# dscripka/openWakeWord

Measured on NVIDIA H100. Metric: 80ms audio-frames/sec (concurrent streams), higher is better.
Workload: dtype f16 operands / f32 accumulate (mel, BN, LayerNorm, sigmoid in f32; heads' first layer as fp16 hi/lo split = f32-grade)

## Files before the change

openwakeword_b200/csrc/cnn_tc_inc.cu:

```cuda
#include "oww_internal.h"
#include "tc_common.cuh"
#include "mel_device.cuh"
#include <cmath>
#include <cstring>
#include <type_traits>

namespace {

constexpr int kIncEpiWarps = 16;
constexpr int kIncThreads = kIncEpiWarps * 32;
constexpr int kIncMaxG = 7;
constexpr int kMelNF = 2;

__device__ __forceinline__ __half2 u32_as_half2(uint32_t v) {
    return __halves2half2(__ushort_as_half((unsigned short)(v & 0xFFFFu)), __ushort_as_half((unsigned short)(v >> 16)));
}

struct IncArgs {
    IncPlan plan;
    const float* mel; const int* mel_count; int64_t mel_stride; int mel_mask; int back;
    const float* w0; const float* s0; const float* b0;
    const uint8_t* wblob;
    const uint4* tails_in; uint4* tails_out;
    float* emb;
    int B;
    const int* live_chunks; int live_min;
    long long* dbg_clock;
    int fused;
    const int16_t* pcm; int64_t pcm_stride;
    int16_t* tail; int* seen; float* mel_rw; int* mel_count_rw;
    const float* mel_window; const float2* mel_twiddle; const int* mel_start; const int* mel_len; const float* mel_w; int mel_kmax;
    float* feat_ring; int64_t feat_stride; int feat_mask; int* feat_count;
    const HeadDev* heads; int n_heads; int max_n_in;
    float* scores; int score_stride;
    int hring_off, hslot_bytes, hns;
    const Gate* gates; int n_gates;
    uint4* gx; LateLay gx_lay;
};

__device__ __forceinline__ int head_rows(int slot_bytes, int K, int D) {
    const int r = (slot_bytes / (D * 4)) & ~3;
    return r < K ? r : K;
}

template <int kNL>
__global__ void __launch_bounds__(kIncThreads, 1) tc_inc_kernel(const __grid_constant__ IncArgs a) {
    extern __shared__ __align__(128) uint8_t smem[];
    const IncPlan& P = a.plan;
    const int NL = kNL ? kNL : P.n_layers;
    const bool fused = kNL == OWW_N_CONV && a.fused;
    const int G = P.G;
    uint64_t* bars = reinterpret_cast<uint64_t*>(smem);
    float* s_l0 = reinterpret_cast<float*>(smem + 704);
    uint4* act0 = reinterpret_cast<uint4*>(smem + 2048);

    const int warp = __shfl_sync(0xffffffffu, (int)(threadIdx.x >> 5), 0);
    const int lane = threadIdx.x & 31;
    const uint32_t bar0 = smem_u32(bars);
    auto wfull = [&](int i) { return bar0 + 8u * i; };
    const uint32_t tails_bar = bar0 + 8u * 2;
    auto hfull = [&](int i) { return bar0 + 8u * (3 + i); };
    auto hempty = [&](int i) { return bar0 + 8u * (7 + i); };

    if (threadIdx.x == 0) {
        for (int i = 0; i < 2; ++i) mbar_init(wfull(i), 1);
        mbar_init(tails_bar, 1);
        for (int i = 0; i < 4; ++i) { mbar_init(hfull(i), 1); mbar_init(hempty(i), kIncEpiWarps); }
        asm volatile("fence.mbarrier_init.release.cluster;" ::: "memory");
    }
    for (int i = threadIdx.x; i < 9 * 24; i += kIncThreads) s_l0[i] = a.w0[i];
    if (threadIdx.x < 24) { s_l0[216 + threadIdx.x] = a.s0[threadIdx.x]; s_l0[240 + threadIdx.x] = a.b0[threadIdx.x]; }
    asm volatile("fence.proxy.async.shared::cta;" ::: "memory");
    __syncthreads();

    auto load_weights = [&](int l) {
        mbar_expect_tx(wfull(l & 1), (uint32_t)P.L[l].w_bytes);
        bulk_g2s(smem_u32(smem + P.L[l].w_smem), a.wblob + P.L[l].w_off, (uint32_t)P.L[l].w_bytes, wfull(l & 1));
    };
    if (threadIdx.x == 0 && (int)blockIdx.x < P.n_groups) { load_weights(1); load_weights(2); }
    pdl_wait();

    int hq_head = 0, hq_layer = 0, hq_row = 0, hchunk_p = 0;
    auto issue_head_chunk = [&]() -> bool {
        if (hq_head >= a.n_heads) return false;
        const HeadDev& H = a.heads[hq_head];
        const int slot = hchunk_p % a.hns;
        mbar_wait(hempty(slot), ((hchunk_p / a.hns) & 1) ^ 1);
        uint32_t bytes; const float* src;
        if (hq_layer == 0) {
            bytes = (uint32_t)(96 * H.dims[1]) * 4u;
            src = H.blob + H.w_off[0] + (int64_t)hq_row * 96 * H.dims[1];
            if (++hq_row == H.n_in) { hq_row = 0; hq_layer = 1; }
        } else {
            const int K = H.dims[hq_layer], D = H.dims[hq_layer + 1];
            const int rows = head_rows(a.hslot_bytes, K, D);
            bytes = ((uint32_t)(min(rows, K - hq_row) * D) * 4u + 15u) & ~15u;
            src = H.blob + H.w_off[hq_layer] + (int64_t)hq_row * D;
            if ((hq_row += rows) >= K) { hq_row = 0; ++hq_layer; }
        }
        if (hq_layer >= H.n_layers) { hq_layer = 0; ++hq_head; }
        mbar_expect_tx(hfull(slot), bytes);
        bulk_g2s(smem_u32(smem + a.hring_off + slot * a.hslot_bytes), src, bytes, hfull(slot));
        ++hchunk_p;
        return true;
    };

    const int et = threadIdx.x;
    uint32_t epar[2] = {0, 0};
    uint32_t epi_tails_par = 0, mma_tails_par = 0;
    uint32_t hf_par = 0; int hchunk_e = 0;
    for (int grp = blockIdx.x; grp < P.n_groups; grp += gridDim.x) {
        const uint4* tin = a.tails_in + (int64_t)grp * P.tail_units;
        uint4* tout = a.tails_out + (int64_t)grp * P.tail_units;
        int* s_cnt = reinterpret_cast<int*>(smem + 512);
        int* s_live = s_cnt + 16;
        float* s_mel = reinterpret_cast<float*>(smem + P.scratch_off + 6144);
        if (a.dbg_clock && blockIdx.x == 0 && grp == 0 && et == 0) a.dbg_clock[101] = clock64();
        named_bar_sync(2, kIncEpiWarps * 32);
        if (et < G) {
            const int b = grp * G + et;
            s_live[et] = b < a.B && (!a.live_chunks || a.live_chunks[b] >= a.live_min);
        }
        named_bar_sync(2, kIncEpiWarps * 32);
        if (fused) {
            uint8_t* sc = smem + P.scratch_off;
            float2* s_tw = reinterpret_cast<float2*>(sc);
            float* s_win = reinterpret_cast<float*>(sc + 4096);
            uint8_t* s_work = smem + 2048 + warp * (kMelNF * kMelFrameScratch);
            float* s_floor = s_mel + G * 256;
            int seen_v = 1;
            for (int i = et; i < 512; i += kIncEpiWarps * 32) { s_tw[i] = a.mel_twiddle[i]; s_win[i] = a.mel_window[i]; }
            if (et < G) {
                const int b = grp * G + et;
                s_cnt[et] = s_live[et] ? a.mel_count_rw[b] : 0;
                s_cnt[8 + et] = s_live[et] ? a.feat_count[b] : 0;
                seen_v = s_live[et] ? a.seen[b] : 1;
                s_live[8 + et] = s_live[et] && seen_v == 0;
            }
            named_bar_sync(2, kIncEpiWarps * 32);
            const int my_start = a.mel_start[lane], my_len = a.mel_len[lane];
            const float* my_w = a.mel_w + lane * OWW_MEL_MAXSUPPORT;
            for (int fi = warp * kMelNF; fi < G * 8; fi += kIncEpiWarps * kMelNF) {
                const int16_t* tl[kMelNF]; const int16_t* bd[kMelNF]; int fr[kMelNF]; float db[kMelNF];
#pragma unroll
                for (int i = 0; i < kMelNF; ++i) {
                    const int fj = fi + i < G * 8 ? fi + i : fi;
                    int b = grp * G + (fj >> 3);
                    if (b >= a.B) b = grp * G;
                    tl[i] = a.tail + (int64_t)b * OWW_TAIL; bd[i] = a.pcm + (int64_t)b * a.pcm_stride; fr[i] = fj & 7;
                }
                long long* st = (a.dbg_clock && blockIdx.x == 0 && grp == 0 && warp == 0 && fi == 0) ? a.dbg_clock + 92 : nullptr;
                mel_frames_db<kMelNF>(tl, OWW_TAIL, bd, fr, s_work, s_tw, s_win, a.mel_kmax, my_start, my_len, my_w, lane, db, st);
#pragma unroll
                for (int i = 0; i < kMelNF; ++i)
                    if (fi + i < G * 8) s_mel[(fi + i) * 32 + lane] = db[i];
            }
            named_bar_sync(2, kIncEpiWarps * 32);
            if (a.dbg_clock && blockIdx.x == 0 && grp == 0 && et == 0) a.dbg_clock[97] = clock64();
            constexpr int kTW = OWW_TAIL / 2;
            const bool al = ((size_t)a.pcm & 3) == 0 && (a.pcm_stride & 1) == 0;
            uint32_t tv[4]; int ti[4];
#pragma unroll
            for (int u = 0; u < 4; ++u) {
                const int i = et + u * kIncEpiWarps * 32;
                ti[u] = -1; tv[u] = 0;
                if (i < G * kTW) {
                    const int g = i / kTW, k = i - g * kTW, b = grp * G + g;
                    if (s_live[g]) {
                        const int16_t* src = a.pcm + (int64_t)b * a.pcm_stride + (OWW_SAMPLES_PER_CHUNK - OWW_TAIL) + 2 * k;
                        tv[u] = al ? __ldg(reinterpret_cast<const uint32_t*>(src))
                                   : ((uint32_t)(unsigned short)__ldg(src) | ((uint32_t)(unsigned short)__ldg(src + 1) << 16));
                        ti[u] = b * kTW + k;
                    }
                }
            }
            if (warp < G) {
                float m = -INFINITY;
                const int j0 = s_live[8 + warp] ? 3 : 0;
#pragma unroll
                for (int j = 0; j < 8; ++j) if (j >= j0) m = fmaxf(m, s_mel[warp * 256 + j * 32 + lane]);
#pragma unroll
                for (int o = 16; o > 0; o >>= 1) m = fmaxf(m, __shfl_xor_sync(0xffffffffu, m, o));
                if (lane == 0) s_floor[warp] = m - 80.0f;
            }
            named_bar_sync(2, kIncEpiWarps * 32);
            for (int i = et; i < G * 256; i += kIncEpiWarps * 32) {
                const int g = i >> 8, b = grp * G + g;
                float v = fmaxf(s_mel[i], s_floor[g]);
                v = v / 10.0f + 2.0f;
                const int fr = (i >> 5) & 7, skip = s_live[8 + g] ? 3 : 0;
                if (fr < skip) v = 1.0f;
                s_mel[i] = v;
                if (s_live[g] && fr >= skip)
                    a.mel_rw[(int64_t)b * a.mel_stride + (int64_t)((s_cnt[g] + fr - skip) & a.mel_mask) * 32 + (i & 31)] = v;
            }
#pragma unroll
            for (int u = 0; u < 4; ++u)
                if (ti[u] >= 0) reinterpret_cast<uint32_t*>(a.tail)[ti[u]] = tv[u];
            static_assert(kIncMaxG * (OWW_TAIL / 2) <= 4 * kIncEpiWarps * 32, "tail copy: four words per thread cover a group");
            if (grp + (int)gridDim.x < P.n_groups && et < G * 20) {
                const int g = et / 20, ln = et - g * 20, b = (grp + (int)gridDim.x) * G + g;
                if (b < a.B) asm volatile("prefetch.global.L2 [%0];" ::"l"(reinterpret_cast<const char*>(a.pcm + (int64_t)b * a.pcm_stride) + ln * 128));
            }
            if (et < G && s_live[et]) {
                const int b = grp * G + et;
                a.mel_count_rw[b] = oww_wrap_count(s_cnt[et] + (s_live[8 + et] ? 5 : 8));
                const int sn = seen_v + 1;
                a.seen[b] = sn > (1 << 30) ? (1 << 30) : sn;
            }
            named_bar_sync(2, kIncEpiWarps * 32);
        }
        for (int l = 0; l < NL; ++l) {
            const IncLayer& L = P.L[l];
            const bool to_global = kNL != OWW_N_CONV && l == NL - 1 && NL < OWW_N_CONV;
            if (a.dbg_clock && blockIdx.x == 0 && grp == 0 && et == 0) a.dbg_clock[l] = clock64();
            uint4* nx = act0 + L.nx_base;
            auto fill_tails_and_guards = [&]() {
                if (L.nx_tail_off >= 0 && et == 0) {
                    const uint32_t per_bytes = (uint32_t)(2 * G * L.nx_Wp) * 16u;
                    mbar_expect_tx(tails_bar, per_bytes * L.cg_out);
                    for (int pl = 0; pl < L.cg_out; ++pl)
                        bulk_g2s(smem_u32(nx + pl * L.nx_pitch + 1), tin + L.nx_tail_off + pl * (2 * G * L.nx_Wp), per_bytes, tails_bar);
                }
                if (!L.final && et < L.cg_out) nx[et * L.nx_pitch] = make_uint4(0, 0, 0, 0);
            };
            if (l > 0 && L.kh3) { mbar_wait(tails_bar, mma_tails_par); mma_tails_par ^= 1; }
            if (!L.pool_t) fill_tails_and_guards();
            else if (et < L.cg_out) (act0 + L.tmp_base)[et * L.tmp_pitch] = make_uint4(0, 0, 0, 0);

            if (l == 0) {
                const int Wp = 33, NP2 = 17;
                for (int q = et; q < 8 * G * NP2; q += kIncEpiWarps * 32) {
                    const int j = q % NP2, tg = q / NP2, g = tg % G, t = tg / G;
                    const int f0 = 2 * j;
                    const int b = grp * G + g;
                    uint4* o = nx + 1 + tg * Wp + f0;
                    const uint4 z = make_uint4(0, 0, 0, 0);
                    if (j == 16) { o[0] = z; o[L.nx_pitch] = z; o[2 * L.nx_pitch] = z; continue; }
                    if (!s_live[g]) {
                        o[0] = z; o[L.nx_pitch] = z; o[2 * L.nx_pitch] = z;
                        o[1] = z; o[L.nx_pitch + 1] = z; o[2 * L.nx_pitch + 1] = z;
                        continue;
                    }
                    const float* base = a.mel + (int64_t)b * a.mel_stride;
                    const int row0 = (fused ? s_cnt[g] - 2 : a.mel_count[b] - a.back - 10) + t;
                    float x[3][4];
#pragma unroll
                    for (int dt = 0; dt < 3; ++dt) {
                        const float* rp = (fused && t + dt >= 2) ? s_mel + (g * 8 + t + dt - 2) * 32
                                                                   : base + (int64_t)((row0 + dt) & a.mel_mask) * 32;
#pragma unroll
                        for (int i = 0; i < 4; ++i) {
                            const int ff = f0 + i - 1;
                            x[dt][i] = (ff >= 0 && ff < 32) ? rp[ff] : 0.f;
                        }
                    }
#pragma unroll
                    for (int pl = 0; pl < 3; ++pl) {
                        __half2 h0[4], h1[4];
#pragma unroll
                        for (int u = 0; u < 4; ++u) {
                            float v0[2], v1[2];
#pragma unroll
                            for (int e = 0; e < 2; ++e) {
                                const int c = pl * 8 + u * 2 + e;
                                float s0 = 0.f, s1 = 0.f;
#pragma unroll
                                for (int k = 0; k < 9; ++k) {
                                    const float w = s_l0[k * 24 + c];
                                    s0 = fmaf(x[k / 3][k % 3], w, s0);
                                    s1 = fmaf(x[k / 3][k % 3 + 1], w, s1);
                                }
                                const float sc = s_l0[216 + c], bi = s_l0[240 + c];
                                v0[e] = act(fmaf(fmaxf(s0, 0.f), sc, bi));
                                v1[e] = act(fmaf(fmaxf(s1, 0.f), sc, bi));
                            }
                            h0[u] = __floats2half2_rn(v0[0], v0[1]);
                            h1[u] = __floats2half2_rn(v1[0], v1[1]);
                        }
                        o[pl * L.nx_pitch] = *reinterpret_cast<uint4*>(h0);
                        o[pl * L.nx_pitch + 1] = *reinterpret_cast<uint4*>(h1);
                    }
                }
            } else {
                mbar_wait(wfull(l & 1), epar[l & 1]);
                epar[l & 1] ^= 1;
                const float* sb = reinterpret_cast<const float*>(smem + L.w_smem + 3 * L.cgp * L.np * 16);
                uint4* dst = L.pool_t ? (act0 + L.tmp_base) : nx;
                const int dpitch = L.pool_t ? L.tmp_pitch : L.nx_pitch;
                const int t_off_units = L.pool_t ? 0 : L.nx_t_off * G * L.Wp;
                const int n_t64 = (L.M + 63) / 64;
                const int tail_start = (L.T_out - 2) * G * L.Wp;
                const uint32_t wp_magic = 0xFFFFFFFFu / (uint32_t)L.Wp + 1u, g_magic = G > 1 ? 0xFFFFFFFFu / (uint32_t)G + 1u : 0u;
                const bool edbg = a.dbg_clock && blockIdx.x == 0 && grp == 0 && et == 0;
                long long e0 = 0;
                if (edbg) e0 = clock64();
                const int wg = warp >> 2, wq = warp & 3, q = lane & 3;
                const uint32_t w_addr = smem_u32(smem + L.w_smem);
                const uint32_t a_base = smem_u32(act0 + L.in_base);
                const int nq = L.cgp / 2;
                const uint32_t a_hi_pair = (uint32_t)make_desc(0, (uint32_t)L.in_pitch * 16u, 128u);
                const uint32_t a_hi_self = (uint32_t)make_desc(0, 0u, 128u);
                const uint64_t dhi = make_desc(0, 0u, 128u) & 0xFFFFFFFF00000000ull;
                const uint32_t b_lo0 = (uint32_t)make_desc(0, (uint32_t)L.np * 16u, 128u);
                const uint32_t a_unit0 = (a_base >> 4) + 1u;
                const uint32_t b_unit0 = w_addr >> 4;
                const uint32_t tap0 = (uint32_t)L.tap[0], tap1 = (uint32_t)L.tap[1], tap2 = (uint32_t)L.tap[2];
                const uint32_t pitch2 = 2u * (uint32_t)L.in_pitch, np2 = 2u * (uint32_t)L.np, tap_w = (uint32_t)(L.cgp * L.np);
                const int n_pair = L.cg_in / 2;
                const bool chained = (L.cg_in & 1) != 0;
                const int n_steps = chained ? 3 * n_pair + 2 : 3 * nq;
                const uint32_t a_cross = (uint32_t)make_desc(0, ((uint32_t)(L.cg_in - 1) * (uint32_t)L.in_pitch + tap0 - tap1) * 16u, 128u);
                const uint32_t last_plane = (uint32_t)(L.cg_in - 1) * (uint32_t)L.in_pitch;
                const int nc = L.np <= 48 ? L.np : L.np / 2;
                const int n_chunks = L.np / nc;
                const int n_items = n_t64 * n_chunks;
                const int lM = L.M, lWp = L.Wp, lW = L.W, lnp = L.np, lcg_out = L.cg_out, ltail = L.nx_tail_off;
                const bool lpool = L.pool_t != 0;
                const uint32_t lin_pitch = (uint32_t)L.in_pitch;
                const int tail_pitch = 2 * G * lWp;
                auto mma_item = [&](auto nc_const, auto ns_const, float* acc, int it) {
                    constexpr int NP = decltype(nc_const)::value;
                    constexpr int NS = decltype(ns_const)::value;
                    constexpr bool kChained = NS % 3 == 2;
                    constexpr int kPair = kChained ? (NS - 2) / 3 : NS / 3, kNq = NS / 3;
                    const int t64 = it / n_chunks, c0 = (it - t64 * n_chunks) * NP;
                    const uint32_t a_t0 = a_unit0 + (uint32_t)(t64 * 64);
                    const uint32_t b_unit = b_unit0 + (uint32_t)c0;
#pragma unroll
                    for (int s = 0; s < NS; ++s) {
                        uint32_t a_off, a_f, b_off;
                        if (kChained) {
                            const int k1 = s - kPair - 1, k2 = s - 2 * kPair - 1;
                            a_off = s < kPair ? tap0 + (uint32_t)s * pitch2
                                  : s == kPair ? tap1
                                  : k1 < kPair ? tap1 + lin_pitch + (uint32_t)k1 * pitch2
                                  : k2 < kPair ? tap2 + (uint32_t)k2 * pitch2
                                  : tap2 + last_plane;
                            a_f = s == kPair ? a_cross : (k2 >= kPair ? a_hi_self : a_hi_pair);
                            b_off = (uint32_t)s * np2;
                        } else {
                            const int j = s / kNq, qq = s - j * kNq;
                            a_off = (j == 0 ? tap0 : j == 1 ? tap1 : tap2) + (uint32_t)qq * pitch2;
                            a_f = a_hi_pair;
                            b_off = (uint32_t)j * tap_w + (uint32_t)qq * np2;
                        }
                        wg_mma<NP>(acc, dhi | a_f | ((a_t0 + a_off) & 0x3FFFu), dhi | b_lo0 | ((b_unit + b_off) & 0x3FFFu), s > 0);
                    }
                };
                auto epi_item = [&](auto nc_const, auto final_const, const float* acc, int it) {
                    constexpr int NP = decltype(nc_const)::value;
                    constexpr bool kFinal = decltype(final_const)::value;
                    const int t64 = it / n_chunks, c0 = (it - t64 * n_chunks) * NP;
#pragma unroll
                    for (int i = 0; i < 2; ++i) {
                        const int m = t64 * 64 + wq * 16 + (lane >> 2) + 8 * i;
                        if (m >= lM) continue;
                        const int tg = (int)__umulhi((uint32_t)m, wp_magic);
                        const int f = m - tg * lWp;
                        const int g = G > 1 ? tg - (int)__umulhi((uint32_t)tg, g_magic) * G : 0;
                        const bool live = s_live[g] != 0;
                        if constexpr (kFinal) {
                            if (f != 0 || !live) continue;
                            float* o = fused ? a.feat_ring + (int64_t)(grp * G + g) * a.feat_stride + (int64_t)(s_cnt[8 + g] & a.feat_mask) * 96
                                               : a.emb + (int64_t)(grp * G + g) * 96;
#pragma unroll
                            for (int j = 0; j < NP / 8; ++j) {
                                const int c = c0 + j * 8 + 2 * q;
                                float2 r;
                                r.x = fmaf(acc[4 * j + 2 * i], sb[c], sb[lnp + c]);
                                r.y = fmaf(acc[4 * j + 2 * i + 1], sb[c + 1], sb[lnp + c + 1]);
                                *reinterpret_cast<float2*>(o + c) = r;
                            }
                            continue;
                        }
                        const bool pad = f == lW;
                        uint4* d0 = dst + (1 + t_off_units + m);
                        const bool keep_tail = !lpool && ltail >= 0 && m >= tail_start && live;
                        uint4* t0 = tout + (ltail + (m - tail_start));
#pragma unroll
                        for (int j = 0; j < NP / 8; ++j) {
                            const int pl = c0 / 8 + j;
                            if (pl >= lcg_out) break;
                            const int c = pl * 8 + 2 * q;
                            const float y0 = act(fmaf(acc[4 * j + 2 * i], sb[c], sb[lnp + c]));
                            const float y1 = act(fmaf(acc[4 * j + 2 * i + 1], sb[c + 1], sb[lnp + c + 1]));
                            const __half2 h = __floats2half2_rn(y0, y1);
                            const uint32_t hw = pad ? 0u : *reinterpret_cast<const uint32_t*>(&h);
                            reinterpret_cast<uint32_t*>(d0 + pl * dpitch)[q] = hw;
                            if (keep_tail) reinterpret_cast<uint32_t*>(t0 + pl * tail_pitch)[q] = hw;
                            if (to_global) {
                                const __half2 lo = __floats2half2_rn(y0 - __low2float(h), y1 - __high2float(h));
                                reinterpret_cast<uint32_t*>(d0 + (lcg_out + pl) * dpitch)[q] = pad ? 0u : *reinterpret_cast<const uint32_t*>(&lo);
                            }
                        }
                    }
                };
                auto run_items = [&](auto nc_const, auto ns_const, auto final_const) {
                    constexpr int NP = decltype(nc_const)::value;
                    for (int it = wg; it < n_items; it += 4) {
                        float acc0[NP / 2];
                        wg_fence();
                        mma_item(nc_const, ns_const, acc0, it);
                        wg_commit();
                        wg_wait_all();
                        if (edbg && it == 0) a.dbg_clock[61 + l] = clock64() - e0;
                        epi_item(nc_const, final_const, acc0, it);
                    }
                };
                using std::integral_constant;
                const std::false_type planes;
                switch (n_steps * 256 + nc) {
                    case 5 * 256 + 32: run_items(integral_constant<int, 32>{}, integral_constant<int, 5>{}, planes); break;
                    case 5 * 256 + 48: run_items(integral_constant<int, 48>{}, integral_constant<int, 5>{}, planes); break;
                    case 9 * 256 + 48: run_items(integral_constant<int, 48>{}, integral_constant<int, 9>{}, planes); break;
                    case 9 * 256 + 40: run_items(integral_constant<int, 40>{}, integral_constant<int, 9>{}, planes); break;
                    case 14 * 256 + 40: run_items(integral_constant<int, 40>{}, integral_constant<int, 14>{}, planes); break;
                    case 14 * 256 + 48: run_items(integral_constant<int, 48>{}, integral_constant<int, 14>{}, planes); break;
                    case 18 * 256 + 48:
                        if (kNL == OWW_N_CONV && L.final) run_items(integral_constant<int, 48>{}, integral_constant<int, 18>{}, std::true_type{});
                        else run_items(integral_constant<int, 48>{}, integral_constant<int, 18>{}, planes);
                        break;
                    default: __trap();
                }
                if (edbg) a.dbg_clock[81 + l] = clock64() - e0;
                if (L.pool_t) {
                    named_bar_sync(2, kIncEpiWarps * 32);
                    if (!to_global) fill_tails_and_guards();
                    if (L.nx_tail_off >= 0 && L.nx_rows_new == 1) {
                        mbar_wait(tails_bar, epi_tails_par);
                        const int perrow = G * L.nx_Wp;
                        for (int i = et; i < L.cg_out * perrow; i += kIncEpiWarps * 32) {
                            const int pl = i / perrow, u = i - pl * perrow;
                            if (s_live[u / L.nx_Wp])
                                tout[L.nx_tail_off + pl * 2 * perrow + u] = nx[pl * L.nx_pitch + 1 + perrow + u];
                        }
                    }
                    const uint4* src = act0 + L.tmp_base;
                    const int T2 = L.T_out / L.pool_t;
                    const int per = T2 * G * L.nx_Wp;
                    const uint32_t per_magic = 0xFFFFFFFFu / (uint32_t)per + 1u, nwp_magic = 0xFFFFFFFFu / (uint32_t)L.nx_Wp + 1u;
                    const uint32_t gp_magic = G > 1 ? 0xFFFFFFFFu / (uint32_t)G + 1u : 0u;
                    for (int i = et; i < L.cg_out * per; i += kIncEpiWarps * 32) {
                        const int pl = per > 1 ? (int)__umulhi((uint32_t)i, per_magic) : i, p = i - pl * per;
                        const int tg = (int)__umulhi((uint32_t)p, nwp_magic), f = p - tg * L.nx_Wp;
                        const int t = G > 1 ? (int)__umulhi((uint32_t)tg, gp_magic) : tg, g = tg - t * G;
                        uint4 res = make_uint4(0, 0, 0, 0);
                        if (to_global) {
                            uint4 res_lo = make_uint4(0, 0, 0, 0);
                            if (f < L.nx_W) {
                                uint32_t bh[4] = {0, 0, 0, 0}, bl[4] = {0, 0, 0, 0};
                                bool first = true;
                                for (int da = 0; da < L.pool_t; ++da)
                                    for (int db = 0; db < L.pool_f; ++db) {
                                        const int at = 1 + ((t * L.pool_t + da) * G + g) * L.Wp + f * L.pool_f + db;
                                        const uint4 q = src[pl * L.tmp_pitch + at], ql = src[(L.cg_out + pl) * L.tmp_pitch + at];
                                        const uint32_t qh[4] = {q.x, q.y, q.z, q.w}, qq[4] = {ql.x, ql.y, ql.z, ql.w};
#pragma unroll
                                        for (int u = 0; u < 4; ++u) {
                                            const __half2 h2 = u32_as_half2(qh[u]), l2 = u32_as_half2(qq[u]);
                                            const __half2 b2 = u32_as_half2(bh[u]), c2 = u32_as_half2(bl[u]);
                                            const uint32_t m = first ? 0xFFFFFFFFu
                                                                     : (__hgt2_mask(h2, b2) | (__heq2_mask(h2, b2) & __hgt2_mask(l2, c2)));
                                            bh[u] = (qh[u] & m) | (bh[u] & ~m);
                                            bl[u] = (qq[u] & m) | (bl[u] & ~m);
                                        }
                                        first = false;
                                    }
                                res = make_uint4(bh[0], bh[1], bh[2], bh[3]);
                                res_lo = make_uint4(bl[0], bl[1], bl[2], bl[3]);
                            }
                            if (s_live[g]) {
                                const int64_t u = late_unit(a.gx_lay, pl, grp * G + g, t, f);
                                a.gx[u] = res;
                                a.gx[u + (int64_t)L.cg_out * a.gx_lay.units] = res_lo;
                            }
                            continue;
                        }
                        if (f < L.nx_W) {
                            __half2 mx[4];
                            bool first = true;
                            for (int da = 0; da < L.pool_t; ++da)
                                for (int db = 0; db < L.pool_f; ++db) {
                                    const uint4 q = src[pl * L.tmp_pitch + 1 + ((t * L.pool_t + da) * G + g) * L.Wp + f * L.pool_f + db];
                                    const __half2* hv = reinterpret_cast<const __half2*>(&q);
#pragma unroll
                                    for (int u = 0; u < 4; ++u) mx[u] = first ? hv[u] : __hmax2(mx[u], hv[u]);
                                    first = false;
                                }
                            res = *reinterpret_cast<uint4*>(mx);
                        }
                        nx[pl * L.nx_pitch + 1 + L.nx_t_off * G * L.nx_Wp + p] = res;
                        if (L.nx_tail_off >= 0 && s_live[g]) {
                            const int keep = T2 >= 2 ? 2 : 1;
                            if (t >= T2 - keep)
                                tout[L.nx_tail_off + pl * (2 * G * L.nx_Wp) + ((2 - keep + t - (T2 - keep)) * G + g) * L.nx_Wp + f] = res;
                        }
                    }
                }
            }
            if (L.nx_tail_off >= 0) epi_tails_par ^= 1;
            asm volatile("fence.proxy.async.shared::cta;" ::: "memory");
            named_bar_sync(1, kIncEpiWarps * 32);
            if (l > 0 && et == 0) {
                if (l + 2 < NL) load_weights(l + 2);
                else if (grp + (int)gridDim.x < P.n_groups) {
                    if (l == NL - 2 && (l & 1)) load_weights(1);
                    if (l == NL - 1) { if (l & 1) load_weights(1); load_weights(2); }
                }
            }
        }
        if (a.dbg_clock && blockIdx.x == 0 && grp == 0 && et == 0) a.dbg_clock[OWW_N_CONV] = clock64();
        if (fused) {
            named_bar_sync(2, kIncEpiWarps * 32);
            if (a.n_heads > 0) {
            if (et == 0) {
                hq_head = hq_layer = hq_row = 0;
                for (int i = 0; i < a.hns && issue_head_chunk(); ++i) {}
            }
            auto refill_head_ring = [&]() {
                while (hchunk_p < hchunk_e - 1 + max(a.hns, 2) && issue_head_chunk()) {}
            };
            const int NI = a.max_n_in;
            float* feats = reinterpret_cast<float*>(smem + 2048);
            float* red = feats + G * NI * 96;
            float* hA = red + 4 * G * 128;
            float* hB = hA + G * 256;
            for (int i0 = et; i0 < G * NI * 24; i0 += 4 * kIncEpiWarps * 32) {
                float4 v[4];
#pragma unroll
                for (int u = 0; u < 4; ++u) {
                    const int i = i0 + u * kIncEpiWarps * 32;
                    v[u] = make_float4(0.f, 0.f, 0.f, 0.f);
                    if (i < G * NI * 24) {
                        const int g = i / (NI * 24), r = (i / 24) % NI, c4 = (i % 24) * 4, b = grp * G + g;
                        if (s_live[g]) {
                            const int row = s_cnt[8 + g] + 1 - NI + r;
                            if (row >= 0) v[u] = __ldcg(reinterpret_cast<const float4*>(a.feat_ring + (int64_t)b * a.feat_stride + (int64_t)(row & a.feat_mask) * 96 + c4));
                        }
                    }
                }
#pragma unroll
                for (int u = 0; u < 4; ++u) {
                    const int i = i0 + u * kIncEpiWarps * 32;
                    if (i < G * NI * 24) *reinterpret_cast<float4*>(feats + i * 4) = v[u];
                }
            }
            named_bar_sync(2, kIncEpiWarps * 32);
            for (int hh = 0; hh < a.n_heads; ++hh) {
                const HeadDev& H = a.heads[hh];
                const int D1 = H.dims[1], off = NI - H.n_in;
                {
                    const int slice = et >> 7, d = et & 127;
                    float acc[kIncMaxG];
#pragma unroll
                    for (int g = 0; g < kIncMaxG; ++g) acc[g] = 0.f;
                    for (int c = 0; c < H.n_in; ++c) {
                        const int slot = hchunk_e % a.hns;
                        mbar_wait(hfull(slot), (hf_par >> slot) & 1u);
                        hf_par ^= 1u << slot;
                        ++hchunk_e;
                        if (d < D1) {
                            const float* wr = reinterpret_cast<const float*>(smem + a.hring_off + slot * a.hslot_bytes) + slice * 24 * D1 + d;
                            const float* xr = feats + (off + c) * 96 + slice * 24;
#pragma unroll 2
                            for (int k4 = 0; k4 < 24; k4 += 4) {
                                const float w0 = wr[(k4 + 0) * D1], w1 = wr[(k4 + 1) * D1];
                                const float w2 = wr[(k4 + 2) * D1], w3 = wr[(k4 + 3) * D1];
#pragma unroll
                                for (int g = 0; g < kIncMaxG; ++g)
                                    if (g < G) {
                                        const float4 x = *reinterpret_cast<const float4*>(xr + g * NI * 96 + k4);
                                        acc[g] = fmaf(x.x, w0, acc[g]);
                                        acc[g] = fmaf(x.y, w1, acc[g]);
                                        acc[g] = fmaf(x.z, w2, acc[g]);
                                        acc[g] = fmaf(x.w, w3, acc[g]);
                                    }
                            }
                        }
                        __syncwarp();
                        if (lane == 0) mbar_arrive(hempty(slot));
                        if (et == 0) refill_head_ring();
                    }
                    if (d < D1) {
#pragma unroll
                        for (int g = 0; g < kIncMaxG; ++g)
                            if (g < G) red[(slice * G + g) * 128 + d] = acc[g];
                    }
                }
                named_bar_sync(2, kIncEpiWarps * 32);
                for (int i = et; i < G * D1; i += kIncEpiWarps * 32) {
                    const int g = i / D1, d = i - g * D1;
                    float v = __ldg(H.blob + H.b_off[0] + d) + red[(0 * G + g) * 128 + d];
                    v += red[(1 * G + g) * 128 + d];
                    v += red[(2 * G + g) * 128 + d];
                    v += red[(3 * G + g) * 128 + d];
                    hA[g * 256 + d] = v;
                }
                named_bar_sync(2, kIncEpiWarps * 32);
                float* cur = hA; float* nxt = hB;
                for (int l = 0; l < H.n_layers; ++l) {
                    const int D = H.dims[l + 1], K = H.dims[l];
                    if (l > 0) {
                        const int rows = head_rows(a.hslot_bytes, K, D);
                        const int nown = min(4, max(0, (G * D - et + kIncEpiWarps * 32 - 1) / (kIncEpiWarps * 32)));
                        float accl[4]; int cxo[4], dd[4];
#pragma unroll
                        for (int j = 0; j < 4; ++j) {
                            const int i = j < nown ? et + j * kIncEpiWarps * 32 : 0;
                            const int g = i / D;
                            dd[j] = i - g * D; cxo[j] = g * 256; accl[j] = 0.f;
                        }
                        for (int k0 = 0; k0 < K; k0 += rows) {
                            const int r = min(rows, K - k0);
                            const int slot = hchunk_e % a.hns;
                            mbar_wait(hfull(slot), (hf_par >> slot) & 1u);
                            hf_par ^= 1u << slot;
                            ++hchunk_e;
                            const float* wr = reinterpret_cast<const float*>(smem + a.hring_off + slot * a.hslot_bytes);
#pragma unroll
                            for (int j = 0; j < 4; ++j) {
                                if (j >= nown) break;
                                const float* cx = cur + cxo[j] + k0;
                                const float* wc = wr + dd[j];
                                float sacc = accl[j];
#pragma unroll 8
                                for (int k = 0; k < r; ++k) sacc = fmaf(cx[k], wc[k * D], sacc);
                                accl[j] = sacc;
                            }
                            __syncwarp();
                            if (lane == 0) mbar_arrive(hempty(slot));
                            if (et == 0) refill_head_ring();
                        }
#pragma unroll
                        for (int j = 0; j < 4; ++j)
                            if (j < nown) nxt[cxo[j] + dd[j]] = accl[j] + __ldg(H.blob + H.b_off[l] + dd[j]);
                        named_bar_sync(2, kIncEpiWarps * 32);
                        float* t = cur; cur = nxt; nxt = t;
                    }
                    if (l < H.n_layers - 1) {
                        if (warp < G) {
                            float* row = cur + warp * 256;
                            if (H.layernorm) {
                                float sum = 0.f;
                                for (int d = lane; d < D; d += 32) sum += row[d];
#pragma unroll
                                for (int o = 16; o > 0; o >>= 1) sum += __shfl_xor_sync(0xffffffffu, sum, o);
                                const float mu = sum / (float)D;
                                float sq = 0.f;
                                for (int d = lane; d < D; d += 32) { const float c = row[d] - mu; sq = fmaf(c, c, sq); }
#pragma unroll
                                for (int o = 16; o > 0; o >>= 1) sq += __shfl_xor_sync(0xffffffffu, sq, o);
                                const float rstd = 1.0f / sqrtf(sq / (float)D + 1e-5f);
                                const float* gm = H.blob + H.g_off[l];
                                const float* hb = H.blob + H.h_off[l];
                                for (int d = lane; d < D; d += 32)
                                    row[d] = fmaxf((row[d] - mu) * rstd * __ldg(gm + d) + __ldg(hb + d), 0.f);
                            } else {
                                for (int d = lane; d < D; d += 32) row[d] = fmaxf(row[d], 0.f);
                            }
                        }
                        named_bar_sync(2, kIncEpiWarps * 32);
                    }
                }
                if (et < G && s_live[et]) {
                    const int n_out = H.dims[H.n_layers];
                    float* row = cur + et * 256;
                    if (H.final_act == 4) {
                        for (int d = 0; d < n_out; ++d) row[d] = fmaxf(row[d], 0.f);
                    } else if (H.final_act == 1) {
                        for (int d = 0; d < n_out; ++d) row[d] = 1.0f / (1.0f + expf(-row[d]));
                    } else if (H.final_act == 2 || H.final_act == 3) {
                        float m = -INFINITY;
                        for (int d = 0; d < n_out; ++d) {
                            if (H.final_act == 3) row[d] = fmaxf(row[d], 0.f);
                            m = fmaxf(m, row[d]);
                        }
                        float sum = 0.f;
                        for (int d = 0; d < n_out; ++d) { row[d] = expf(row[d] - m); sum += row[d]; }
                        for (int d = 0; d < n_out; ++d) row[d] = row[d] / sum;
                    }
                    float* o = a.scores + (int64_t)(grp * G + et) * a.score_stride + H.col0;
                    for (int d = 0; d < n_out; ++d) o[d] = row[d];
                }
                named_bar_sync(2, kIncEpiWarps * 32);
            }
            }
            if (et < G && s_live[et]) {
                if (a.n_heads > 0) {
                    float* o = a.scores + (int64_t)(grp * G + et) * a.score_stride;
                    for (int q = 0; q < a.n_gates; ++q)
                        if (o[a.gates[q].main_col] > a.gates[q].thr) o[a.gates[q].main_col] = o[a.gates[q].ver_col];
                }
                a.feat_count[grp * G + et] = oww_wrap_count(s_cnt[8 + et] + 1);
            }
            named_bar_sync(2, kIncEpiWarps * 32);
            if (a.dbg_clock && blockIdx.x == 0 && grp == 0 && et == 0) a.dbg_clock[102] = clock64();
        }
    }
}

__global__ void __launch_bounds__(256) tc_capture_kernel(const uint4* planes, int64_t plane_pitch, int T, int Wp, int cg,
                                                         int win0, int n_win, int stream0, const int* ids, int G, int tail_off,
                                                         int tail_units, uint4* tails) {
    const int per = 2 * Wp;
    const int64_t total = (int64_t)n_win * cg * per;
    for (int64_t i = (int64_t)blockIdx.x * 256 + threadIdx.x; i < total; i += (int64_t)gridDim.x * 256) {
        const int u = (int)(i % per);
        const int pl = (int)((i / per) % cg);
        const int w = (int)(i / ((int64_t)per * cg));
        const int r = u / Wp, f = u - r * Wp;
        const int b = ids ? ids[stream0 + w] : stream0 + w, grp = b / G, g = b - grp * G;
        const uint4 v = planes[(int64_t)pl * plane_pitch + kGuard + (int64_t)(win0 + w) * T * Wp + (int64_t)(T - 2 + r) * Wp + f];
        tails[(int64_t)grp * tail_units + tail_off + pl * (2 * G * Wp) + (r * G + g) * Wp + f] = v;
    }
}

}

int oww_inc_build_plan(oww_ctx* ctx, int G, int n_streams, int n_layers, IncPlan* out) {
    if (G < 1 || G > kIncMaxG) return oww_fail(ctx, OWW_EINVAL, "group size must be 1..%d", kIncMaxG);
    const int NL = n_layers;
    if (NL < 3 || NL > OWW_N_CONV || (NL < OWW_N_CONV && !ctx->conv[NL - 1].pool_t))
        return oww_fail(ctx, OWW_EINVAL, "fused-CNN plan: cannot cut after layer %d", NL - 1);
    constexpr int kTop = 227 * 1024;
    constexpr int kActBase = 2048;
    IncPlan P;
    std::memset(&P, 0, sizeof(P));
    P.G = G;
    P.n_groups = (n_streams + G - 1) / G;
    P.n_layers = NL;
    for (int l = 0; l < OWW_N_CONV; ++l) P.L[l].nx_tail_off = -1;
    int rows_new = 8, W = 32;
    int tail_units = 0;
    int x_units = 0, y_units = 0;
    size_t w_off = 0;
    auto pitch_of = [&](int rows, int wp) { return (1 + rows * G * wp + 7) & ~7; };
    auto need = [&](int buf, int units) { if (buf) { if (units > y_units) y_units = units; } else { if (units > x_units) x_units = units; } };
    int cur_buf = 0;
    int use_x[OWW_N_CONV] = {0}, use_y[OWW_N_CONV] = {0};
    for (int l = 0; l < NL; ++l) {
        const ConvLayer& C = ctx->conv[l];
        IncLayer& L = P.L[l];
        const bool cut = l == NL - 1 && NL < OWW_N_CONV;
        L.final = l == OWW_N_CONV - 1;
        L.kh3 = C.kh == 3 && l > 0;
        L.W = W; L.Wp = W + 1;
        L.cg_in = C.cin / 8; L.cgp = (L.cg_in + 1) & ~1; L.np = (C.cout + 15) & ~15; L.cg_out = C.cout / 8;
        L.pool_t = C.pool_t; L.pool_f = C.pool_f;
        auto use = [&](int buf, int units) { need(buf, units); int& u = buf ? use_y[l] : use_x[l]; if (units > u) u = units; };
        if (l == 0) {
            L.T_out = 8; L.M = 0;
        } else {
            L.in_buf = cur_buf;
            L.rows_in = rows_new + (L.kh3 ? 2 : 0);
            L.T_out = rows_new;
            L.M = L.T_out * G * L.Wp;
            L.in_pitch = P.L[l - 1].nx_pitch;
            use(L.in_buf, L.in_pitch * L.cg_in);
            if (L.kh3) { L.tap[0] = 0; L.tap[1] = G * L.Wp; L.tap[2] = 2 * G * L.Wp; }
            else { L.tap[0] = -1; L.tap[1] = 0; L.tap[2] = 1; }
            L.w_off = (int)w_off;
            L.w_bytes = 3 * L.cgp * L.np * 16 + 2 * L.np * 4;
            w_off += (size_t)((L.w_bytes + 127) & ~127);
        }
        const bool next_kh3 = !cut && l + 1 < OWW_N_CONV && ctx->conv[l + 1].kh == 3;
        int nrows = L.T_out, nW = W;
        if (L.pool_t) { nrows = L.T_out / L.pool_t; nW = W / L.pool_f; }
        L.nx_W = nW; L.nx_Wp = nW + 1; L.nx_rows_new = nrows;
        L.nx_t_off = (next_kh3 && !L.final) ? 2 : 0;
        L.out_buf = l == 0 ? 0 : (cur_buf ^ 1);
        L.nx_buf = (l == 0) ? 0 : (L.pool_t ? cur_buf : L.out_buf);
        L.nx_pitch = pitch_of(nrows + L.nx_t_off, L.nx_Wp);
        if (L.pool_t) { L.tmp_pitch = pitch_of(L.T_out, L.Wp); use(L.out_buf, L.tmp_pitch * L.cg_out * (cut ? 2 : 1)); }
        if (!L.final && !cut) use(L.nx_buf, L.nx_pitch * L.cg_out);
        L.nx_tail_off = -1;
        if (L.nx_t_off == 2) { L.nx_tail_off = tail_units; tail_units += L.cg_out * 2 * G * L.nx_Wp; }
        cur_buf = L.nx_buf;
        rows_new = nrows; W = nW;
    }
    P.tail_units = tail_units;
    P.x_units = (x_units + 7) & ~7; P.y_units = (y_units + 7) & ~7;
    int size_nx[OWW_N_CONV] = {0}, size_tmp[OWW_N_CONV] = {0}, xlive[OWW_N_CONV + 1];
    for (int l = 0; l < NL; ++l) {
        const IncLayer& L = P.L[l];
        const bool cut = l == NL - 1 && NL < OWW_N_CONV;
        size_nx[l] = (L.final || cut) ? 0 : L.nx_pitch * L.cg_out;
        size_tmp[l] = L.pool_t ? L.tmp_pitch * L.cg_out * (cut ? 2 : 1) : 0;
    }
    for (int l = 0; l <= OWW_N_CONV; ++l) xlive[l] = 0;
    for (int l = 0; l < NL; ++l) {
        const IncLayer& L = P.L[l];
        auto upd = [&](int cls, int sz) { if (cls == 0 && sz > xlive[l]) xlive[l] = sz; };
        if (l > 0) upd(L.in_buf, size_nx[l - 1]);
        if (L.pool_t) upd(L.out_buf, size_tmp[l]);
        upd(L.nx_buf, size_nx[l]);
    }
    auto r8 = [](int v) { return (v + 7) & ~7; };
    int act_high[OWW_N_CONV] = {0};
    for (int l = 0; l < NL; ++l) {
        IncLayer& L = P.L[l];
        L.in_base = l > 0 ? P.L[l - 1].nx_base : 0;
        L.tmp_base = (L.pool_t && L.out_buf == 1) ? r8(xlive[l]) : 0;
        L.nx_base = L.nx_buf == 1 ? r8(xlive[l] > xlive[l + 1] ? xlive[l] : xlive[l + 1]) : 0;
        int hi = 0;
        if (l > 0 && L.in_base + size_nx[l - 1] > hi) hi = L.in_base + size_nx[l - 1];
        if (L.pool_t && L.tmp_base + size_tmp[l] > hi) hi = L.tmp_base + size_tmp[l];
        if (L.nx_base + size_nx[l] > hi) hi = L.nx_base + size_nx[l];
        act_high[l] = kActBase + hi * 16;
    }
    auto wsz = [&](int l) { return l >= 1 && l < NL ? (P.L[l].w_bytes + 127) & ~127 : 0; };
    for (int l = 1; l < NL; ++l) {
        const int above = wsz(l + 1) > wsz(l - 1) ? wsz(l + 1) : wsz(l - 1);
        P.L[l].w_smem = (l & 1) ? kTop - wsz(l) : kTop - above - wsz(l);
    }
    for (int l = 1; l < NL; ++l) {
        int w_low = P.L[l].w_smem;
        if (l + 1 < NL && P.L[l + 1].w_smem < w_low) w_low = P.L[l + 1].w_smem;
        if (act_high[l] > w_low || act_high[l - 1] > P.L[l].w_smem)
            return oww_fail(ctx, OWW_EUNSUPPORTED, "fused-CNN smem plan does not fit at layer %d (G=%d)", l, G);
        if (l >= 2 && wsz(l) < wsz(l - 1)) return oww_fail(ctx, OWW_EUNSUPPORTED, "weight sizes must not shrink with depth");
    }
    if (NL == OWW_N_CONV) {
        int off = kActBase + r8(size_nx[0]) * 16;
        const int work_end = kActBase + kIncEpiWarps * kMelNF * kMelFrameScratch;
        if (work_end > off) off = (work_end + 127) & ~127;
        const int need_b = 6144 + G * 256 * 4 + 64;
        P.scratch_off = (off + need_b <= P.L[1].w_smem && off + need_b <= P.L[2].w_smem) ? off : 0;
    }
    P.w_total_bytes = (int)w_off;
    P.smem_bytes = kTop;
    *out = P;
    return OWW_OK;
}

int oww_inc_setup(oww_ctx* ctx, const float* h_blob) {
    IncPlan P;
    int rc = oww_inc_build_plan(ctx, 1, 1, OWW_N_CONV, &P);
    if (rc) return rc;
    std::vector<uint8_t> blob(P.w_total_bytes, 0);
    size_t off = 0;
    for (int li = 0; li < OWW_N_CONV; ++li) {
        const ConvLayer& C = ctx->conv[li];
        const size_t nw = (size_t)C.kh * C.kw * C.cin * C.cout;
        const float* w = h_blob + off; const float* sc = w + nw; const float* bi = sc + C.cout;
        off += nw + 2 * (size_t)C.cout;
        if (li == 0) continue;
        const IncLayer& L = P.L[li];
        const int sexp = oww_weight_scale_exponent(w, nw);
        const float up = std::ldexp(1.0f, sexp), down = std::ldexp(1.0f, -sexp);
        __half* hw = reinterpret_cast<__half*>(blob.data() + L.w_off);
        const int cg = L.cg_in;
        auto octet_at = [&](int j, int g) {
            if (!(cg & 1)) return j * L.cgp + g;
            if (j == 0) return g < cg - 1 ? g : cg;
            if (j == 1) return g == 0 ? cg - 1 : cg + g;
            return 2 * cg + g;
        };
        for (int j = 0; j < 3; ++j)
            for (int g = 0; g < cg; ++g)
                for (int n = 0; n < L.np; ++n)
                    for (int e = 0; e < 8; ++e) {
                        const int c = g * 8 + e;
                        const float v = (c < C.cin && n < C.cout) ? w[((size_t)j * C.cin + c) * C.cout + n] : 0.f;
                        hw[(((size_t)octet_at(j, g)) * L.np + n) * 8 + e] = __float2half_rn(v * up);
                    }
        float* sb = reinterpret_cast<float*>(blob.data() + L.w_off + (size_t)3 * L.cgp * L.np * 16);
        for (int n = 0; n < L.np; ++n) { sb[n] = n < C.cout ? sc[n] * down : 0.f; sb[L.np + n] = n < C.cout ? bi[n] : 0.f; }
    }
    if (!ctx->d_inc_w) OWW_CUDA(ctx, cudaMalloc(&ctx->d_inc_w, blob.size()));
    OWW_CUDA(ctx, cudaMemcpy(ctx->d_inc_w, blob.data(), blob.size(), cudaMemcpyHostToDevice));
    return OWW_OK;
}

int oww_inc_n_layers(const oww_ctx* ctx) {
    return (ctx->cfg.cnn_mode == OWW_CNN_TC_INCREMENTAL && ctx->split_from < OWW_N_CONV) ? ctx->split_from : OWW_N_CONV;
}

int oww_inc_alloc_streams(oww_ctx* ctx) {
    int best_g = 0; double best_cost = 0;
    for (int g = 1; g <= kIncMaxG; ++g) {
        IncPlan P;
        if (oww_inc_build_plan(ctx, g, ctx->n_streams, oww_inc_n_layers(ctx), &P) != OWW_OK) continue;
        const int rounds = (P.n_groups + ctx->sm_count - 1) / ctx->sm_count;
        const double cost = rounds * (50.0 + 6.5 * g);
        if (!best_g || cost < best_cost) { best_g = g; best_cost = cost; }
    }
    if (!best_g) return oww_fail(ctx, OWW_EUNSUPPORTED, "no feasible group size for the fused CNN kernel");
    ctx->err.clear();
    int rc = oww_inc_build_plan(ctx, best_g, ctx->n_streams, oww_inc_n_layers(ctx), &ctx->inc_plan);
    if (rc) return rc;
    const size_t bytes = (size_t)ctx->inc_plan.n_groups * ctx->inc_plan.tail_units * 16;
    for (int i = 0; i < 2; ++i) {
        cudaFree(ctx->d_inc_tails[i]); ctx->d_inc_tails[i] = nullptr;
        OWW_CUDA(ctx, cudaMalloc(&ctx->d_inc_tails[i], bytes));
        OWW_CUDA(ctx, cudaMemset(ctx->d_inc_tails[i], 0, bytes));
    }
    ctx->inc_cur = 0;
    ctx->tails_template_valid = false;
    OWW_CUDA(ctx, cudaFuncSetAttribute(tc_inc_kernel<OWW_N_CONV>, cudaFuncAttributeMaxDynamicSharedMemorySize, ctx->inc_plan.smem_bytes));
    OWW_CUDA(ctx, cudaFuncSetAttribute(tc_inc_kernel<11>, cudaFuncAttributeMaxDynamicSharedMemorySize, ctx->inc_plan.smem_bytes));
    OWW_CUDA(ctx, cudaFuncSetAttribute(tc_inc_kernel<15>, cudaFuncAttributeMaxDynamicSharedMemorySize, ctx->inc_plan.smem_bytes));
    OWW_CUDA(ctx, cudaFuncSetAttribute(tc_inc_kernel<0>, cudaFuncAttributeMaxDynamicSharedMemorySize, ctx->inc_plan.smem_bytes));
    return OWW_OK;
}

int oww_heads_sync_devs(oww_ctx* ctx) {
    std::vector<HeadDev> v(ctx->heads.size());
    for (size_t i = 0; i < ctx->heads.size(); ++i) {
        const Head& h = ctx->heads[i];
        HeadDev& d = v[i];
        std::memset(&d, 0, sizeof(d));
        d.blob = h.d_blob;
        d.n_in = h.desc.n_in; d.n_layers = h.desc.n_layers; d.layernorm = h.desc.layernorm; d.final_act = h.desc.final_act;
        for (int l = 0; l <= h.desc.n_layers; ++l) d.dims[l] = h.desc.dims[l];
        for (int l = 0; l < h.desc.n_layers; ++l) {
            d.w_off[l] = (int)h.w_off[l]; d.b_off[l] = (int)h.b_off[l];
            d.g_off[l] = (int)h.g_off[l]; d.h_off[l] = (int)h.h_off[l];
        }
        d.col0 = h.col0;
    }
    cudaFree(ctx->d_head_devs); ctx->d_head_devs = nullptr;
    if (v.empty()) return OWW_OK;
    OWW_CUDA(ctx, cudaMalloc(&ctx->d_head_devs, v.size() * sizeof(HeadDev)));
    OWW_CUDA(ctx, cudaMemcpy(ctx->d_head_devs, v.data(), v.size() * sizeof(HeadDev), cudaMemcpyHostToDevice));
    return OWW_OK;
}

bool oww_fused_frontend_supported(const oww_ctx* ctx) {
    return ctx->fuse_step && ctx->cfg.cnn_mode == OWW_CNN_TC_INCREMENTAL &&
           (ctx->inc_plan.n_layers < OWW_N_CONV || ctx->inc_plan.scratch_off != 0);
}

bool oww_fused_heads_supported(const oww_ctx* ctx) {
    if (!oww_fused_frontend_supported(ctx) || ctx->heads.empty() || ctx->heads.size() > 16) return false;
    if (ctx->inc_plan.n_layers < OWW_N_CONV) return false;
    {
        size_t w1 = 0;
        for (const Head& h : ctx->heads) w1 += (size_t)h.desc.dims[0] * h.desc.dims[1] * sizeof(float);
        if ((size_t)ctx->inc_plan.n_groups * w1 > ((size_t)256 << 20)) return false;
    }
    for (const Head& h : ctx->heads) {
        if (h.desc.dims[1] > 128) return false;
        for (int l = 1; l <= h.desc.n_layers; ++l) if (h.desc.dims[l] > 256) return false;
    }
    const size_t floats = (size_t)ctx->inc_plan.G * ((size_t)ctx->max_n_in * 96 + 4 * 128 + 2 * 256);
    int d1max = 32;
    for (const Head& h : ctx->heads) d1max = h.desc.dims[1] > d1max ? h.desc.dims[1] : d1max;
    return 2048 + floats * 4 + 128 + (size_t)96 * d1max * 4 <= (size_t)ctx->inc_plan.L[2].w_smem;
}

static cudaError_t launch_inc(const IncArgs& a, int grid, cudaStream_t s, bool pdl = false) {
    void (*k)(IncArgs) = a.plan.n_layers == OWW_N_CONV ? tc_inc_kernel<OWW_N_CONV>
                       : a.plan.n_layers == 11         ? tc_inc_kernel<11>
                       : a.plan.n_layers == 15         ? tc_inc_kernel<15>
                                                       : tc_inc_kernel<0>;
    return oww_launch_pdl(pdl, k, dim3(grid), dim3(kIncThreads), (size_t)a.plan.smem_bytes, s, a);
}

static void fill_inc_args(oww_ctx* ctx, IncArgs& a) {
    std::memset(&a, 0, sizeof(a));
    a.plan = ctx->inc_plan;
    a.mel = ctx->d_mel_ring; a.mel_count = ctx->d_mel_count; a.mel_stride = (int64_t)ctx->mel_rows * 32;
    a.mel_mask = ctx->mel_rows - 1;
    a.w0 = ctx->conv[0].d_w; a.s0 = ctx->conv[0].d_scale; a.b0 = ctx->conv[0].d_bias;
    a.wblob = reinterpret_cast<const uint8_t*>(ctx->d_inc_w);
    a.tails_in = reinterpret_cast<const uint4*>(ctx->d_inc_tails[ctx->inc_cur]);
    a.tails_out = reinterpret_cast<uint4*>(ctx->d_inc_tails[ctx->inc_cur ^ 1]);
    a.B = ctx->n_streams;
    a.dbg_clock = reinterpret_cast<long long*>(ctx->d_inc_dbg);
    if (ctx->late_active) {
        a.gx = reinterpret_cast<uint4*>(ctx->late_x[ctx->split_from].buf[0]);
        a.gx_lay = ctx->late_x[ctx->split_from].lay;
    }
}

int oww_fused_step(oww_ctx* ctx, const int16_t* d_pcm, int64_t pcm_stride, float* d_scores, int out_stride, bool with_heads,
                   cudaStream_t s, const int* d_chunks, int min_chunks) {
    IncArgs a;
    fill_inc_args(ctx, a);
    a.live_chunks = d_chunks; a.live_min = min_chunks;
    const int grid = a.plan.n_groups < ctx->sm_count ? a.plan.n_groups : ctx->sm_count;
    if (a.plan.n_layers < OWW_N_CONV) {
        MelLaunch m{d_pcm, pcm_stride, OWW_SAMPLES_PER_CHUNK, ctx->d_tail, ctx->d_seen, ctx->d_mel_ring,
                    (int64_t)ctx->mel_rows * 32, ctx->mel_rows - 1, ctx->d_mel_count, ctx->n_streams, 1, 1};
        m.live = d_chunks; m.live_min = min_chunks; m.pdl = ctx->late_pdl;
        int rc = oww_mel_launch(ctx, m, s);
        if (rc) return rc;
        OWW_CUDA(ctx, launch_inc(a, grid, s, ctx->late_pdl));
        OWW_LAUNCH_CHECK(ctx);
        ctx->inc_cur ^= 1;
        return OWW_OK;
    }
    a.fused = 1;
    a.pcm = d_pcm; a.pcm_stride = pcm_stride;
    a.tail = ctx->d_tail; a.seen = ctx->d_seen; a.mel_rw = ctx->d_mel_ring; a.mel_count_rw = ctx->d_mel_count;
    a.mel_window = ctx->d_window; a.mel_twiddle = ctx->d_twiddle; a.mel_start = ctx->d_mel_start; a.mel_len = ctx->d_mel_len;
    a.mel_w = ctx->d_mel_w; a.mel_kmax = ctx->mel_kmax;
    a.feat_ring = ctx->d_feat_ring; a.feat_stride = (int64_t)ctx->feat_rows * 96; a.feat_mask = ctx->feat_rows - 1;
    a.feat_count = ctx->d_feat_count;
    a.heads = ctx->d_head_devs; a.n_heads = with_heads ? (int)ctx->heads.size() : 0; a.max_n_in = ctx->max_n_in > 0 ? ctx->max_n_in : 1;
    a.scores = d_scores; a.score_stride = out_stride;
    a.gates = ctx->d_gates; a.n_gates = with_heads ? (int)ctx->gates.size() : 0;
    if (with_heads) {
        int d1max = 32;
        for (const Head& h : ctx->heads) d1max = h.desc.dims[1] > d1max ? h.desc.dims[1] : d1max;
        const int G = a.plan.G;
        const int used = 2048 + (G * (a.max_n_in * 96 + 4 * 128 + 2 * 256)) * 4;
        a.hring_off = (used + 127) & ~127;
        a.hslot_bytes = 96 * d1max * 4;
        const int avail = a.plan.L[2].w_smem - a.hring_off;
        a.hns = avail / a.hslot_bytes;
        if (a.hns > 4) a.hns = 4;
        if (a.hns < 1 && !ctx->heads.empty()) return oww_fail(ctx, OWW_EUNSUPPORTED, "no room for the fused heads weight ring");
    }
    OWW_CUDA(ctx, launch_inc(a, grid, s));
    OWW_LAUNCH_CHECK(ctx);
    ctx->inc_cur ^= 1;
    return OWW_OK;
}

int oww_cnn_inc_step(oww_ctx* ctx, int back, float* d_emb, cudaStream_t s, const int* d_chunks, int min_chunks) {
    IncArgs a;
    fill_inc_args(ctx, a);
    a.live_chunks = d_chunks; a.live_min = min_chunks;
    a.back = back;
    a.emb = d_emb;
    const int grid = a.plan.n_groups < ctx->sm_count ? a.plan.n_groups : ctx->sm_count;
    OWW_CUDA(ctx, launch_inc(a, grid, s));
    OWW_LAUNCH_CHECK(ctx);
    ctx->inc_cur ^= 1;
    if (ctx->late_active) return oww_late_chain(ctx, d_emb, s);
    return OWW_OK;
}

int oww_inc_capture(oww_ctx* ctx, int layer, const void* planes, int64_t plane_pitch, int T, int W, int win0, int n_win,
                    int stream0, const int* d_ids, cudaStream_t s) {
    const IncLayer& L = ctx->inc_plan.L[layer];
    if (layer >= ctx->inc_plan.n_layers - (ctx->inc_plan.n_layers < OWW_N_CONV ? 1 : 0) || L.nx_tail_off < 0) return OWW_OK;
    const int Wp = W + 1;
    const int64_t total = (int64_t)n_win * L.cg_out * 2 * Wp;
    unsigned grid = (unsigned)((total + 255) / 256);
    tc_capture_kernel<<<grid, 256, 0, s>>>(reinterpret_cast<const uint4*>(planes), plane_pitch, T, Wp, L.cg_out, win0, n_win,
                                          stream0, d_ids, ctx->inc_plan.G, L.nx_tail_off, ctx->inc_plan.tail_units,
                                          reinterpret_cast<uint4*>(ctx->d_inc_tails[ctx->inc_cur]));
    OWW_LAUNCH_CHECK(ctx);
    return OWW_OK;
}

namespace {
__global__ void fill_ones_kernel(float* p, int n) {
    const int i = blockIdx.x * blockDim.x + threadIdx.x;
    if (i < n) p[i] = 1.0f;
}
}

int oww_inc_build_template(oww_ctx* ctx) {
    if (!ctx->emb_loaded) return oww_fail(ctx, OWW_EINVAL, "embedding weights not loaded");
    if (!ctx->d_tc_act[0] || !ctx->d_inc_tails[0]) return oww_fail(ctx, OWW_EINVAL, "oww_set_streams has not been called");
    IncPlan P1;
    int rc = oww_inc_build_plan(ctx, 1, 1, ctx->inc_plan.n_layers, &P1);
    if (rc) return rc;
    ctx->n_tail_tab = 0;
    for (int l = 0; l < OWW_N_CONV; ++l)
        if (P1.L[l].nx_tail_off >= 0)
            ctx->tail_tab[ctx->n_tail_tab++] = make_int4(P1.L[l].nx_tail_off, ctx->inc_plan.L[l].nx_tail_off, P1.L[l].cg_out, P1.L[l].nx_Wp);
    cudaFree(ctx->d_tails_template); ctx->d_tails_template = nullptr;
    OWW_CUDA(ctx, cudaMalloc(&ctx->d_tails_template, (size_t)P1.tail_units * 16));
    OWW_CUDA(ctx, cudaMemset(ctx->d_tails_template, 0, (size_t)P1.tail_units * 16));
    float* d_ones = nullptr; float* d_emb = nullptr;
    OWW_CUDA(ctx, cudaMalloc(&d_ones, OWW_WINDOW_ROWS * 32 * sizeof(float)));
    OWW_CUDA(ctx, cudaMalloc(&d_emb, 96 * sizeof(float)));
    fill_ones_kernel<<<(OWW_WINDOW_ROWS * 32 + 255) / 256, 256>>>(d_ones, OWW_WINDOW_ROWS * 32);
    const IncPlan saved_plan = ctx->inc_plan;
    void* const saved_tails = ctx->d_inc_tails[ctx->inc_cur];
    ctx->inc_plan = P1;
    ctx->d_inc_tails[ctx->inc_cur] = ctx->d_tails_template;
    WindowSrc src{d_ones, (int64_t)OWW_WINDOW_ROWS * 32, nullptr, -1, 0, 0};
    TailCapture cap{0, 1, 0};
    cap.late = ctx->late_active;
    rc = oww_cnn_tc_pyramid_cap(ctx, src, 1, d_emb, &cap, nullptr);
    cudaError_t e = cudaDeviceSynchronize();
    ctx->inc_plan = saved_plan;
    ctx->d_inc_tails[ctx->inc_cur] = saved_tails;
    cudaFree(d_ones); cudaFree(d_emb);
    if (rc) return rc;
    if (e != cudaSuccess) return oww_fail(ctx, OWW_ECUDA, "tails template: %s", cudaGetErrorString(e));
    ctx->tails_template_valid = true;
    return OWW_OK;
}
```

openwakeword_b200/csrc/mel.cu:

```cuda
#include "oww_internal.h"
#include "tc_common.cuh"
#include "mel_device.cuh"
#include <climits>
#include <cmath>
#include <cstring>

namespace {

constexpr int kWarps = 8;
constexpr int kThreads = kWarps * 32;

struct MelDev {
    const float* window;
    const float2* twiddle;
    const int* mel_start;
    const int* mel_len;
    const float* mel_w;
    int kmax;
};

__global__ void __launch_bounds__(kThreads, 5) mel_kernel(MelLaunch p, MelDev c) {
    __shared__ __align__(16) uint8_t s_work[kWarps][kMelFrameScratch];
    __shared__ float2 s_tw[512];
    __shared__ float s_win[512];
    __shared__ float s_red[kWarps];

    pdl_trigger();
    const int clip = p.ids ? p.ids[blockIdx.x] : blockIdx.x;
    const int tid = threadIdx.x, lane = tid & 31, warp = tid >> 5;
    if (p.live && p.live[clip] < p.live_min) {
        pdl_wait();
        return;
    }

    for (int i = tid; i < 512; i += kThreads) { s_tw[i] = c.twiddle[i]; s_win[i] = c.window[i]; }

    const bool streaming = p.tail != nullptr;
    const int prefix = streaming ? OWW_TAIL : 0;
    const int seen0 = streaming ? p.seen[clip] : 0;
    const bool fresh = streaming && seen0 == 0;
    const int total = prefix + p.n_body;
    const int T = (total - OWW_FFT_N) / OWW_HOP + 1;
    const int f0 = fresh ? 3 : 0;
    const int nrows = T - f0;
    const bool one_pass = nrows <= kWarps;
    const int16_t* body = p.body + (int64_t)clip * p.body_stride;
    const int16_t* tail = streaming ? p.tail + (int64_t)clip * OWW_TAIL : nullptr;
    const int row0 = p.out_count ? p.out_count[clip] : 0;
    float* out = p.out + (int64_t)clip * p.out_stride;
    __syncthreads();

    const int my_start = c.mel_start[lane];
    const int my_len = c.mel_len[lane];
    const float* my_w = c.mel_w + lane * OWW_MEL_MAXSUPPORT;
    float vmax = -INFINITY, kept = 0.f;

    for (int f = f0 + warp; f < T; f += kWarps) {
        float db;
        mel_frames_db<1>(&tail, prefix, &body, &f, s_work[warp], s_tw, s_win, c.kmax, my_start, my_len, my_w, lane, &db);
        vmax = fmaxf(vmax, db);
        if (one_pass) { kept = db; continue; }
        pdl_wait();
        const int r = f - f0;
        const int slot = p.out_rows_mask >= 0 ? ((row0 + r) & p.out_rows_mask) : r;
        out[(int64_t)slot * OWW_MEL_BINS + lane] = db;
    }
#pragma unroll
    for (int o = 16; o > 0; o >>= 1) vmax = fmaxf(vmax, __shfl_xor_sync(0xffffffffu, vmax, o));
    if (lane == 0) s_red[warp] = vmax;
    __syncthreads();
    float m = s_red[0];
#pragma unroll
    for (int w = 1; w < kWarps; ++w) m = fmaxf(m, s_red[w]);
    const float floor_db = m - 80.0f;
    int16_t tv[(OWW_TAIL + kThreads - 1) / kThreads];
#pragma unroll
    for (int u = 0; u < (OWW_TAIL + kThreads - 1) / kThreads; ++u) {
        const int i = tid + u * kThreads;
        tv[u] = streaming && i < OWW_TAIL ? __ldg(body + (p.n_body - OWW_TAIL + i)) : (int16_t)0;
    }
    pdl_wait();
    if (one_pass) {
        if (warp < nrows) {
            float v = fmaxf(kept, floor_db);
            if (p.affine) v = v / 10.0f + 2.0f;
            const int slot = p.out_rows_mask >= 0 ? ((row0 + warp) & p.out_rows_mask) : warp;
            out[(int64_t)slot * OWW_MEL_BINS + lane] = v;
        }
    } else {
        for (int i = tid; i < nrows * OWW_MEL_BINS; i += kThreads) {
            const int r = i >> 5, col = i & 31;
            const int slot = p.out_rows_mask >= 0 ? ((row0 + r) & p.out_rows_mask) : r;
            float* q = out + (int64_t)slot * OWW_MEL_BINS + col;
            float v = fmaxf(__ldcg(q), floor_db);
            if (p.affine) v = v / 10.0f + 2.0f;
            *q = v;
        }
    }
    if (streaming) {
        int16_t* tw = p.tail + (int64_t)clip * OWW_TAIL;
#pragma unroll
        for (int u = 0; u < (OWW_TAIL + kThreads - 1) / kThreads; ++u)
            if (tid + u * kThreads < OWW_TAIL) tw[tid + u * kThreads] = tv[u];
        if (tid == 0) {
            p.out_count[clip] = oww_wrap_count(row0 + nrows);
            const int sn = seen0 + p.n_chunks;
            p.seen[clip] = sn > (1 << 30) ? (1 << 30) : sn;
        }
    }
}

__host__ __device__ __forceinline__ int clip_frame_step(int f) { return f < 5 ? 0 : (f - 5) / 8 + 1; }
__host__ __device__ __forceinline__ int clip_group(int f, int chunk) {
    return (int)oww_call_first_step(oww_call_of_step(clip_frame_step(f), chunk), chunk);
}
__host__ __device__ __forceinline__ int clip_first_group(int k0, int chunk) { return clip_group(8 * k0 > 71 ? 8 * k0 - 71 : 0, chunk); }

__global__ void __launch_bounds__(kThreads) mel_clip_kernel(const int16_t* pcm, const int64_t* clip_off, const int* clip_len, int pad,
                                                            int chunk, int k0, int k1, float* out, int64_t out_stride, MelDev c) {
    extern __shared__ __align__(16) uint8_t dyn[];
    float2 (*s_buf)[2][256] = reinterpret_cast<float2 (*)[2][256]>(dyn);
    float2* s_tw = reinterpret_cast<float2*>(dyn + kWarps * 2 * 256 * sizeof(float2));
    float* s_win = reinterpret_cast<float*>(s_tw + 512);
    float (*s_pow)[264] = reinterpret_cast<float (*)[264]>(s_win + 512);
    int16_t (*s_frame)[512] = reinterpret_cast<int16_t (*)[512]>(s_pow + kWarps);
    int* s_gmax = reinterpret_cast<int*>(s_frame + kWarps);
    const int clip = blockIdx.x;
    const int tid = threadIdx.x, lane = tid & 31, warp = tid >> 5;
    const int v0 = 8 * k0;
    const int g0 = clip_first_group(k0, chunk);
    const int f0 = g0 == 0 ? 0 : 8 * g0 - 3;
    const int n_frames = 8 * k1 - 3;
    for (int i = tid; i < 512; i += kThreads) { s_tw[i] = c.twiddle[i]; s_win[i] = c.window[i]; }
    for (int i = tid; i < k1 - g0; i += kThreads) s_gmax[i] = INT_MIN;
    const int16_t* body = pcm + clip_off[clip];
    const int n_samples = clip_len[clip];
    float* o = out + (int64_t)clip * out_stride;
    for (int i = tid; i < (71 - v0) * 32; i += kThreads) o[i] = 1.0f;
    __syncthreads();
    const int my_start = c.mel_start[lane];
    const int my_len = c.mel_len[lane];
    const float* my_w = c.mel_w + lane * OWW_MEL_MAXSUPPORT;
    auto enc = [](float v) { int i = __float_as_int(v); return i >= 0 ? i : i ^ 0x7FFFFFFF; };
    for (int f = f0 + warp; f < n_frames; f += kWarps) {
        for (int j = lane; j < 512; j += 32) {
            const int64_t p = (int64_t)f * OWW_HOP + j - pad;
            s_frame[warp][j] = (p >= 0 && p < n_samples) ? body[p] : (int16_t)0;
        }
        __syncwarp();
        const float db = mel_frame_db<false>(nullptr, 0, s_frame[warp], 0, s_buf[warp][0], s_buf[warp][1], s_pow[warp], s_tw, s_win, c.kmax,
                                      my_start, my_len, my_w, lane);
        if (71 + f >= v0) o[(int64_t)(71 + f - v0) * 32 + lane] = db;
        float m = db;
#pragma unroll
        for (int k = 16; k > 0; k >>= 1) m = fmaxf(m, __shfl_xor_sync(0xffffffffu, m, k));
        if (lane == 0) atomicMax(&s_gmax[clip_group(f, chunk) - g0], enc(m));
        __syncwarp();
    }
    __syncthreads();
    const int fw = max(f0, v0 - 71);
    for (int i = tid; i < (n_frames - fw) * 32; i += kThreads) {
        const int f = fw + (i >> 5);
        const int e = s_gmax[clip_group(f, chunk) - g0];
        const float gmax = __int_as_float(e >= 0 ? e : e ^ 0x7FFFFFFF);
        float* q = o + (int64_t)(71 + f - v0) * 32 + (i & 31);
        *q = fmaxf(*q, gmax - 80.0f) / 10.0f + 2.0f;
    }
}

double hz_to_mel(double f) {
    const double f_sp = 200.0 / 3.0, min_log_hz = 1000.0, min_log_mel = min_log_hz / f_sp;
    const double logstep = std::log(6.4) / 27.0;
    return f >= min_log_hz ? min_log_mel + std::log(f / min_log_hz) / logstep : f / f_sp;
}
double mel_to_hz(double m) {
    const double f_sp = 200.0 / 3.0, min_log_hz = 1000.0, min_log_mel = min_log_hz / f_sp;
    const double logstep = std::log(6.4) / 27.0;
    return m >= min_log_mel ? min_log_hz * std::exp(logstep * (m - min_log_mel)) : f_sp * m;
}

}

int oww_mel_launch(oww_ctx* ctx, const MelLaunch& p, cudaStream_t s) {
    if (!ctx->mel_loaded) return oww_fail(ctx, OWW_EINVAL, "mel constants not loaded");
    const int prefix = p.tail ? OWW_TAIL : 0;
    if (prefix + p.n_body < OWW_FFT_N) return oww_fail(ctx, OWW_EINVAL, "clip shorter than 512 samples");
    if (p.n_clips <= 0) return OWW_OK;
    MelDev c{ctx->d_window, ctx->d_twiddle, ctx->d_mel_start, ctx->d_mel_len, ctx->d_mel_w, ctx->mel_kmax};
    OWW_CUDA(ctx, oww_launch_pdl(p.pdl, mel_kernel, dim3(p.n_clips), dim3(kThreads), 0, s, p, c));
    OWW_LAUNCH_CHECK(ctx);
    return OWW_OK;
}

int oww_mel_clips_launch(oww_ctx* ctx, const int16_t* d_pcm, const int64_t* d_off, const int* d_len, int n_clips, int pad,
                         int chunk, int k0, int k1, float* d_out, int64_t out_stride, cudaStream_t s) {
    if (!ctx->mel_loaded) return oww_fail(ctx, OWW_EINVAL, "mel constants not loaded");
    if (n_clips <= 0 || k1 <= k0) return OWW_OK;
    if (k0 < 0 || k1 - k0 > 8192 || chunk < 1 || oww_call_first_step(oww_call_of_step(k1, chunk), chunk) != k1)
        return oww_fail(ctx, OWW_EINVAL, "step range [%d,%d) is not a bulk frontend segment", k0, k1);
    MelDev c{ctx->d_window, ctx->d_twiddle, ctx->d_mel_start, ctx->d_mel_len, ctx->d_mel_w, ctx->mel_kmax};
    const size_t smem = (size_t)kWarps * 2 * 256 * sizeof(float2) + 512 * sizeof(float2) + 512 * sizeof(float) +
                        (size_t)kWarps * 264 * sizeof(float) + (size_t)kWarps * 512 * sizeof(int16_t) +
                        (size_t)(k1 - clip_first_group(k0, chunk)) * sizeof(int);
    if (!ctx->mel_clip_attr_set) {
        OWW_CUDA(ctx, cudaFuncSetAttribute(mel_clip_kernel, cudaFuncAttributeMaxDynamicSharedMemorySize, 100 * 1024));
        ctx->mel_clip_attr_set = true;
    }
    mel_clip_kernel<<<n_clips, kThreads, smem, s>>>(d_pcm, d_off, d_len, pad, chunk, k0, k1, d_out, out_stride, c);
    OWW_LAUNCH_CHECK(ctx);
    return OWW_OK;
}

extern "C" int oww_load_mel(oww_ctx* ctx, const float* h_window512, const float* h_mel_fb) {
    if (!ctx) return OWW_EINVAL;
    OWW_CUDA(ctx, cudaSetDevice(ctx->device));
    const double kPi = 3.14159265358979323846;
    std::vector<float> win(512, 0.f);
    if (h_window512) {
        std::memcpy(win.data(), h_window512, 512 * sizeof(float));
    } else {
        for (int n = 0; n < 400; ++n) win[56 + n] = (float)(0.5 - 0.5 * std::cos(2.0 * kPi * n / 400.0));
    }
    std::vector<float2> tw(512);
    for (int k = 0; k < 512; ++k) {
        const double a = -2.0 * kPi * k / 512.0;
        tw[k] = make_float2((float)std::cos(a), (float)std::sin(a));
    }
    std::vector<float> fb(OWW_N_BINS * OWW_MEL_BINS);
    if (h_mel_fb) {
        std::memcpy(fb.data(), h_mel_fb, fb.size() * sizeof(float));
    } else {
        const int n_mels = OWW_MEL_BINS;
        std::vector<double> mel_f(n_mels + 2);
        const double m0 = hz_to_mel(60.0), m1 = hz_to_mel(3800.0);
        for (int i = 0; i < n_mels + 2; ++i) mel_f[i] = mel_to_hz(m0 + (m1 - m0) * i / (n_mels + 1));
        for (int k = 0; k < OWW_N_BINS; ++k) {
            const double ff = 8000.0 * k / 256.0;
            for (int i = 0; i < n_mels; ++i) {
                const double lower = (ff - mel_f[i]) / (mel_f[i + 1] - mel_f[i]);
                const double upper = (mel_f[i + 2] - ff) / (mel_f[i + 2] - mel_f[i + 1]);
                double w = lower < upper ? lower : upper;
                if (w < 0) w = 0;
                w *= 2.0 / (mel_f[i + 2] - mel_f[i]);
                fb[k * n_mels + i] = (float)w;
            }
        }
    }
    std::vector<int> st(OWW_MEL_BINS, 0), ln(OWW_MEL_BINS, 0);
    std::vector<float> mw(OWW_MEL_BINS * OWW_MEL_MAXSUPPORT, 0.f);
    int kmax = 0;
    for (int i = 0; i < OWW_MEL_BINS; ++i) {
        int lo = -1, hi = -1;
        for (int k = 0; k < OWW_N_BINS; ++k)
            if (fb[k * OWW_MEL_BINS + i] != 0.f) { if (lo < 0) lo = k; hi = k; }
        if (lo < 0) { st[i] = 0; ln[i] = 0; continue; }
        if (hi - lo + 1 > OWW_MEL_MAXSUPPORT)
            return oww_fail(ctx, OWW_EUNSUPPORTED, "mel filter %d spans %d FFT bins (max %d)", i, hi - lo + 1,
                            OWW_MEL_MAXSUPPORT);
        st[i] = lo; ln[i] = hi - lo + 1;
        for (int k = lo; k <= hi; ++k) mw[i * OWW_MEL_MAXSUPPORT + (k - lo)] = fb[k * OWW_MEL_BINS + i];
        if (hi + 1 > kmax) kmax = hi + 1;
    }
    ctx->mel_kmax = kmax;
    ctx->mel_key = oww_fnv1a(fb.data(), fb.size() * sizeof(float), oww_fnv1a(win.data(), win.size() * sizeof(float)));
    auto up = [&](void** d, const void* h, size_t bytes) -> cudaError_t {
        if (!*d) { cudaError_t e = cudaMalloc(d, bytes); if (e != cudaSuccess) return e; }
        return cudaMemcpy(*d, h, bytes, cudaMemcpyHostToDevice);
    };
    OWW_CUDA(ctx, up((void**)&ctx->d_window, win.data(), 512 * sizeof(float)));
    OWW_CUDA(ctx, up((void**)&ctx->d_twiddle, tw.data(), 512 * sizeof(float2)));
    OWW_CUDA(ctx, up((void**)&ctx->d_mel_start, st.data(), OWW_MEL_BINS * sizeof(int)));
    OWW_CUDA(ctx, up((void**)&ctx->d_mel_len, ln.data(), OWW_MEL_BINS * sizeof(int)));
    OWW_CUDA(ctx, up((void**)&ctx->d_mel_w, mw.data(), mw.size() * sizeof(float)));
    ctx->mel_loaded = true;
    return OWW_OK;
}
```

openwakeword_b200/csrc/mel_device.cuh:

```cuda
#pragma once
#include <cuda_runtime.h>
#include <cstdint>
#include "oww_internal.h"

namespace {

__device__ __forceinline__ float2 cmul(float2 a, float2 b) {
    return make_float2(__fmaf_rn(a.x, b.x, -__fmul_rn(a.y, b.y)), __fmaf_rn(a.x, b.y, __fmul_rn(a.y, b.x)));
}

template <bool kBodyGlobal = true>
__device__ __forceinline__ float mel_frame_db(const int16_t* tail, int prefix, const int16_t* body, int f, float2* a, float2* b,
                                              float* pw_buf, const float2* s_tw, const float* s_win, int kmax, int my_start,
                                              int my_len, const float* my_w, int lane) {
#pragma unroll
        for (int j = 0; j < 8; ++j) {
            const int n = lane + 32 * j;
            const int s0 = f * OWW_HOP + 2 * n;
            float x0, x1;
            if (s0 + 1 < prefix) { x0 = (float)tail[s0]; x1 = (float)tail[s0 + 1]; }
            else if (s0 >= prefix) {
                if (kBodyGlobal) { x0 = (float)__ldg(body + (s0 - prefix)); x1 = (float)__ldg(body + (s0 + 1 - prefix)); }
                else { x0 = (float)body[s0 - prefix]; x1 = (float)body[s0 + 1 - prefix]; }
            }
            else { x0 = (float)tail[s0]; x1 = kBodyGlobal ? (float)__ldg(body) : (float)body[0]; }
            a[n] = make_float2(__fmul_rn(x0, s_win[2 * n]), __fmul_rn(x1, s_win[2 * n + 1]));
        }
        __syncwarp();
#pragma unroll
        for (int Ns = 1; Ns < 256; Ns *= 4) {
            const int tstep = 128 / Ns;
#pragma unroll
            for (int jj = 0; jj < 2; ++jj) {
                const int j = lane + 32 * jj;
                const int k = j & (Ns - 1);
                float2 v0 = a[j];
                float2 v1 = cmul(a[j + 64], s_tw[k * tstep]);
                float2 v2 = cmul(a[j + 128], s_tw[2 * k * tstep]);
                float2 v3 = cmul(a[j + 192], s_tw[3 * k * tstep]);
                float2 a0 = make_float2(v0.x + v2.x, v0.y + v2.y);
                float2 a1 = make_float2(v0.x - v2.x, v0.y - v2.y);
                float2 a2 = make_float2(v1.x + v3.x, v1.y + v3.y);
                float2 d = make_float2(v1.x - v3.x, v1.y - v3.y);
                float2 a3 = make_float2(d.y, -d.x);
                const int dst = (j / Ns) * Ns * 4 + k;
                b[dst] = make_float2(a0.x + a2.x, a0.y + a2.y);
                b[dst + Ns] = make_float2(a1.x + a3.x, a1.y + a3.y);
                b[dst + 2 * Ns] = make_float2(a0.x - a2.x, a0.y - a2.y);
                b[dst + 3 * Ns] = make_float2(a1.x - a3.x, a1.y - a3.y);
            }
            __syncwarp();
            float2* t = a; a = b; b = t;
        }
        for (int k = lane; k < kmax; k += 32) {
            float pw;
            if (k == 256) {
                const float x = a[0].x - a[0].y;
                pw = __fmul_rn(x, x);
            } else {
                const float2 zk = a[k & 255];
                const float2 zc = a[(256 - k) & 255];
                const float2 xe = make_float2(0.5f * (zk.x + zc.x), 0.5f * (zk.y - zc.y));
                const float2 dd = make_float2(zk.x - zc.x, zk.y + zc.y);
                const float2 xo = make_float2(0.5f * dd.y, -0.5f * dd.x);
                const float2 t2 = cmul(s_tw[k], xo);
                const float re = __fadd_rn(xe.x, t2.x), im = __fadd_rn(xe.y, t2.y);
                pw = __fmaf_rn(re, re, __fmul_rn(im, im));
            }
            pw_buf[k] = pw;
        }
        __syncwarp();
        float acc = 0.f;
        for (int i = 0; i < my_len; ++i) acc = fmaf(pw_buf[my_start + i], my_w[i], acc);
        const float db = 10.0f * logf(fmaxf(acc, 1e-10f)) / logf(10.0f);
    return db;
}

#ifndef OWW_FFT_SWZ
#define OWW_FFT_SWZ 1
#endif
__device__ __forceinline__ int fswz(int e) {
#if OWW_FFT_SWZ
    return e ^ (((e >> 4) & 3) * 5);
#else
    return e;
#endif
}

constexpr int kMelFrameScratch = 2048 + 2048;
template <int NF>
__device__ __forceinline__ void mel_frames_db(const int16_t* const* tail, int prefix, const int16_t* const* body, const int* f,
                                              uint8_t* bufs, const float2* s_tw, const float* s_win, int kmax, int my_start,
                                              int my_len, const float* my_w, int lane, float* db, long long* stamps = nullptr) {
    float2* a[NF]; float2* b[NF]; float* pw[NF];
    if (stamps && lane == 0) stamps[0] = clock64();
#pragma unroll
    for (int i = 0; i < NF; ++i) {
        a[i] = reinterpret_cast<float2*>(bufs + i * kMelFrameScratch);
        b[i] = a[i] + 256;
        pw[i] = reinterpret_cast<float*>(b[i]);
    }
    bool al[NF];
#pragma unroll
    for (int i = 0; i < NF; ++i) al[i] = (((size_t)body[i] | (size_t)tail[i]) & 3) == 0 && (prefix & 1) == 0;
    uint32_t raw[8][NF];
#pragma unroll
    for (int j = 0; j < 8; ++j) {
        const int n = lane + 32 * j;
#pragma unroll
        for (int i = 0; i < NF; ++i) {
            const int s0 = f[i] * OWW_HOP + 2 * n;
            if (al[i]) {
                raw[j][i] = s0 + 1 < prefix ? *reinterpret_cast<const uint32_t*>(tail[i] + s0)
                                            : __ldg(reinterpret_cast<const uint32_t*>(body[i] + (s0 - prefix)));
            } else {
                unsigned short u0, u1;
                if (s0 + 1 < prefix) { u0 = (unsigned short)tail[i][s0]; u1 = (unsigned short)tail[i][s0 + 1]; }
                else if (s0 >= prefix) { u0 = (unsigned short)__ldg(body[i] + (s0 - prefix)); u1 = (unsigned short)__ldg(body[i] + (s0 + 1 - prefix)); }
                else { u0 = (unsigned short)tail[i][s0]; u1 = (unsigned short)__ldg(body[i]); }
                raw[j][i] = (uint32_t)u0 | ((uint32_t)u1 << 16);
            }
        }
    }
#pragma unroll
    for (int j = 0; j < 8; ++j) {
        const int n = lane + 32 * j;
        const float2 wn = *reinterpret_cast<const float2*>(s_win + 2 * n);
#pragma unroll
        for (int i = 0; i < NF; ++i) {
            const float x0 = (float)(short)(raw[j][i] & 0xFFFFu), x1 = (float)(short)(raw[j][i] >> 16);
            a[i][fswz(n)] = make_float2(__fmul_rn(x0, wn.x), __fmul_rn(x1, wn.y));
        }
    }
    __syncwarp();
    if (stamps && lane == 0) stamps[1] = clock64();
#pragma unroll
    for (int Ns = 1; Ns < 256; Ns *= 4) {
        const int tstep = 128 / Ns;
        float2 t1 = make_float2(1.f, 0.f), t2 = t1, t3 = t1;
        if (Ns > 1 && Ns <= 32) { const int k = lane & (Ns - 1); t1 = s_tw[k * tstep]; t2 = s_tw[2 * k * tstep]; t3 = s_tw[3 * k * tstep]; }
#pragma unroll
        for (int jj = 0; jj < 2; ++jj) {
            const int j = lane + 32 * jj;
            const int k = j & (Ns - 1);
            if (Ns > 32) { t1 = s_tw[k * tstep]; t2 = s_tw[2 * k * tstep]; t3 = s_tw[3 * k * tstep]; }
            const int dst = (j / Ns) * Ns * 4 + k;
            const int sj = fswz(j);
            const int d0 = fswz(dst), d1 = fswz(dst + Ns), d2 = fswz(dst + 2 * Ns), d3 = fswz(dst + 3 * Ns);
#pragma unroll
            for (int i = 0; i < NF; ++i) {
                const float2 v0 = a[i][sj];
                float2 v1 = a[i][sj + 64], v2 = a[i][sj + 128], v3 = a[i][sj + 192];
                if (Ns > 1) { v1 = cmul(v1, t1); v2 = cmul(v2, t2); v3 = cmul(v3, t3); }
                float2 a0 = make_float2(v0.x + v2.x, v0.y + v2.y);
                float2 a1 = make_float2(v0.x - v2.x, v0.y - v2.y);
                float2 a2 = make_float2(v1.x + v3.x, v1.y + v3.y);
                float2 d = make_float2(v1.x - v3.x, v1.y - v3.y);
                float2 a3 = make_float2(d.y, -d.x);
                b[i][d0] = make_float2(a0.x + a2.x, a0.y + a2.y);
                b[i][d1] = make_float2(a1.x + a3.x, a1.y + a3.y);
                b[i][d2] = make_float2(a0.x - a2.x, a0.y - a2.y);
                b[i][d3] = make_float2(a1.x - a3.x, a1.y - a3.y);
            }
        }
        __syncwarp();
#pragma unroll
        for (int i = 0; i < NF; ++i) { float2* t = a[i]; a[i] = b[i]; b[i] = t; }
    }
    if (stamps && lane == 0) stamps[2] = clock64();
    for (int k = lane; k < kmax; k += 32) {
#pragma unroll
        for (int i = 0; i < NF; ++i) {
            float p;
            if (k == 256) {
                const float x = a[i][fswz(0)].x - a[i][fswz(0)].y;
                p = __fmul_rn(x, x);
            } else {
                const float2 zk = a[i][fswz(k & 255)];
                const float2 zc = a[i][fswz((256 - k) & 255)];
                const float2 xe = make_float2(0.5f * (zk.x + zc.x), 0.5f * (zk.y - zc.y));
                const float2 dd = make_float2(zk.x - zc.x, zk.y + zc.y);
                const float2 xo = make_float2(0.5f * dd.y, -0.5f * dd.x);
                const float2 t2 = cmul(s_tw[k], xo);
                const float re = __fadd_rn(xe.x, t2.x), im = __fadd_rn(xe.y, t2.y);
                p = __fmaf_rn(re, re, __fmul_rn(im, im));
            }
            pw[i][k] = p;
        }
    }
    __syncwarp();
    if (stamps && lane == 0) stamps[3] = clock64();
    float acc[NF];
#pragma unroll
    for (int i = 0; i < NF; ++i) acc[i] = 0.f;
    for (int q = 0; q < my_len; q += 4) {
        const float4 w4 = __ldg(reinterpret_cast<const float4*>(my_w + q));
        const float w[4] = {w4.x, w4.y, w4.z, w4.w};
#pragma unroll
        for (int e = 0; e < 4; ++e)
            if (q + e < my_len) {
#pragma unroll
                for (int i = 0; i < NF; ++i) acc[i] = fmaf(pw[i][my_start + q + e], w[e], acc[i]);
            }
    }
#pragma unroll
    for (int i = 0; i < NF; ++i) db[i] = 10.0f * logf(fmaxf(acc[i], 1e-10f)) / logf(10.0f);
    __syncwarp();
    if (stamps && lane == 0) stamps[4] = clock64();
}

}
```

openwakeword_b200/csrc/oww_internal.h:

```cpp
#pragma once
#include <cuda_runtime.h>
#include <algorithm>
#include <cmath>
#include <cstdint>
#include <cstdio>
#include <string>
#include <utility>
#include <vector>
#include "owwb200.h"

__host__ __device__ inline int oww_scale_exponent_of_max(float amax, int lo = -8, int hi = 24) {
    if (!(amax > 0.f) || !(amax <= 3.402823466e38f)) return 0;
    int e;
    frexpf(amax, &e);
    e = 14 - e;
    return e < lo ? lo : (e > hi ? hi : e);
}
inline int oww_weight_scale_exponent(const float* w, size_t n) {
    float amax = 0.f;
    for (size_t i = 0; i < n; ++i) amax = std::fmax(amax, std::fabs(w[i]));
    return oww_scale_exponent_of_max(amax);
}

#define OWW_N_CONV 20
#define OWW_FFT_N 512
#define OWW_N_BINS 257
#define OWW_HOP 160
#define OWW_TAIL 480
#define OWW_MEL_MAXSUPPORT 32

struct ConvLayer {
    int kh, kw, cin, cout, pool_t, pool_f;
    int t_in, f_in;
    int t_out, f_out;
    float* d_w;
    float* d_scale;
    float* d_bias;
};

struct Head {
    oww_head_desc desc;
    int n_out;
    int col0;
    float* d_blob;
    std::vector<size_t> w_off, b_off, g_off, h_off;
    struct TcLayer { int K, D, Kp, NP; uint32_t w_off, w_bytes; float unscale; };
    bool tc_ok = false;
    void* d_w1_tc = nullptr;
    std::vector<TcLayer> tc_layers;
    std::vector<float> tc_w0_host;
};

struct LateLay {
    int S, T, Wq, kh3;
    int units;
    int64_t blk_stride;
};
#ifdef __CUDACC__
__host__ __device__ __forceinline__ int64_t late_unit(const LateLay& L, int plane, int stream, int row, int f) {
    const int blk = stream / L.S, sl = stream - blk * L.S;
    const int within = L.kh3 ? (row * L.S + sl) * L.Wq + f : 1 + (sl * L.T + row) * L.Wq + f;
    return (int64_t)blk * L.blk_stride + (int64_t)plane * L.units + within;
}
#endif

struct ResetLate {
    uint4* now;
    uint4* next;
    const uint4* tmpl;
    int Wp, n_planes;
    int off;
    LateLay lay;
};
struct ResetTails { uint4* tails; const uint4* tmpl; int G, tail_units, n_tab; int4 tab[OWW_N_CONV]; int n_late; ResetLate late[OWW_N_CONV]; };

struct Gate { int main_col, ver_col; float thr; };

struct VerifierBank {
    int head_id, col0, n_cols, n_in, capacity;
    int head_bank = -1;
    float thr;
    float* d_mean = nullptr;
    float* d_weight = nullptr;
    float* d_bias = nullptr;
    int* d_assign = nullptr;
    int clip_slot = -1;
};

struct HeadBank {
    Head shape;
    int capacity = 0;
    size_t w_bytes = 0;
    size_t p_floats = 0;
    std::vector<int> p_off;
    uint8_t* d_w = nullptr;
    float* d_p = nullptr;
    void* d_slots = nullptr;
    std::vector<uint8_t> h_slots;
    std::vector<uint8_t> loaded;
    int clip_slot = -1;
    std::vector<int> assign;
    int n_items = 0;
    int* d_table = nullptr;
    int* h_stage = nullptr;
    cudaEvent_t stage_ev = nullptr;
};

#define OWW_COUNT_WRAP (1 << 30)
#define OWW_COUNT_REBASE ((1 << 30) - (1 << 20))
#ifdef __CUDACC__
__device__ __forceinline__ int oww_wrap_count(int c) { return c >= OWW_COUNT_WRAP ? c - OWW_COUNT_REBASE : c; }
#endif

struct HeadDev {
    const float* blob;
    int n_in, n_layers, layernorm, final_act;
    int dims[OWW_MAX_HEAD_LAYERS + 1];
    int w_off[OWW_MAX_HEAD_LAYERS], b_off[OWW_MAX_HEAD_LAYERS], g_off[OWW_MAX_HEAD_LAYERS], h_off[OWW_MAX_HEAD_LAYERS];
    int col0;
};

struct IncLayer {
    int kh3, final;
    int W, Wp;
    int rows_in, T_out, M;
    int cg_in, cgp, np, cg_out;
    int in_buf, out_buf;
    int in_base, tmp_base, nx_base;
    int in_pitch;
    int tap[3];
    int pool_t, pool_f, tmp_pitch;
    int nx_buf, nx_pitch, nx_W, nx_Wp, nx_rows_new, nx_t_off, nx_tail_off;
    int w_off, w_bytes, w_smem;
};
struct IncPlan {
    int G, n_groups, tail_units, x_units, y_units, w_total_bytes, smem_bytes;
    int scratch_off;
    IncLayer L[OWW_N_CONV];
    int n_layers;
};

struct oww_ctx {
    oww_config cfg;
    int device = 0;
    int sm_count = 132;
    std::string err;
    uint64_t launches = 0;

    bool mel_loaded = false;
    float* d_window = nullptr;
    float2* d_twiddle = nullptr;
    int* d_mel_start = nullptr;
    int* d_mel_len = nullptr;
    float* d_mel_w = nullptr;
    int mel_kmax = 0;

    bool emb_loaded = false;
    ConvLayer conv[OWW_N_CONV];
    float* d_emb_blob = nullptr;

    std::vector<Head> heads;
    std::vector<HeadBank> head_banks;
    int n_out_total = 0;
    int max_n_in = 0;
    std::vector<Gate> gates;
    Gate* d_gates = nullptr;
    float* d_scores_tmp = nullptr;
    size_t scores_tmp_floats = 0;
    std::vector<VerifierBank> banks;
    int* d_assign_stage = nullptr;
    bool verifiers_on = true;
    cudaEvent_t ver_ev[2] = {nullptr, nullptr};
    double* d_fit_scratch = nullptr;
    size_t fit_scratch_doubles = 0;
    int64_t* d_fit_off = nullptr;
    size_t fit_off_cap = 0;
    int* d_load_slots = nullptr;
    size_t load_slots_cap = 0;
    bool fit_attr_set = false;

    int n_streams = 0;
    int mel_rows = 128;
    int feat_rows = 128;
    int16_t* d_tail = nullptr;
    int* d_seen = nullptr;
    int* d_mel_count = nullptr;
    int* d_feat_count = nullptr;
    float* d_mel_ring = nullptr;
    float* d_feat_ring = nullptr;

    int window_batch = 256;
    float* d_act[2] = {nullptr, nullptr};
    size_t act_floats = 0;
    float* d_emb_tmp = nullptr;
    size_t emb_tmp_floats = 0;

    void* d_tc_w = nullptr;
    float* d_tc_sb = nullptr;
    void* d_tc_w3 = nullptr;
    float* d_tc_sb3 = nullptr;
    int split_from = 11;
    size_t tc_w_off[OWW_N_CONV] = {0};
    size_t tc_sb_off[OWW_N_CONV] = {0};
    void* d_tc_act[2] = {nullptr, nullptr};
    size_t tc_act_units = 0;

    void* d_inc_w = nullptr;
    void* d_inc_tails[2] = {nullptr, nullptr};
    int inc_cur = 0;
    struct LateTensor { void* buf[3] = {nullptr, nullptr, nullptr}; int n_buf = 0, rows_new = 0, W = 0, cg = 0, tmpl_off = -1;
                        LateLay lay = {0, 0, 0, 0, 0, 0}; };
    LateTensor late_x[OWW_N_CONV];
    void* d_late_tmp = nullptr;
    void* d_late_template = nullptr;
    bool late_active = false;
    bool late_pdl = true;
    long late_step = 0;

    void* d_tails_template = nullptr;
    bool tails_template_valid = false;
    int4 tail_tab[OWW_N_CONV];
    int n_tail_tab = 0;
    int* d_reset_ids = nullptr;
    float* d_reset_init = nullptr;

    uint64_t mel_key = 0, emb_key = 0;
    int* d_state_ids = nullptr;
    int* d_state_rejected = nullptr;
    cudaEvent_t state_ev[2] = {nullptr, nullptr};
    IncPlan inc_plan;
    void* d_inc_dbg = nullptr;
    HeadDev* d_head_devs = nullptr;
    bool fuse_step = true;

    cudaStream_t own_stream = nullptr;
    cudaStream_t copy_stream = nullptr;
    struct HostSlot {
        int16_t* h_pcm = nullptr; int16_t* d_pcm = nullptr; size_t pcm_bytes = 0;
        float* h_scores = nullptr; float* d_scores = nullptr; size_t sc_bytes = 0;
        cudaEvent_t h2d_done = nullptr, done = nullptr;
        bool busy = false;
    } slot[2];
    int next_slot = 0;
    std::vector<int32_t> slot_chunks[2];

    static constexpr int kRagSlots = 4;
    int32_t* h_rag[kRagSlots] = {nullptr, nullptr, nullptr, nullptr};
    int32_t* d_rag[kRagSlots] = {nullptr, nullptr, nullptr, nullptr};
    cudaEvent_t rag_ev[kRagSlots] = {nullptr, nullptr, nullptr, nullptr};
    int rag_next = 0, rag_streams = 0;
    float* d_rag_scores = nullptr;
    size_t rag_scores_floats = 0;

    bool timing = false;
    std::vector<cudaEvent_t> ev;
    std::vector<uint8_t> ev_fused;
    int ev_slots = 0;
    long ev_steps = 0;

    bool heads_attr_set = false;
    bool heads_tc_attr_set = false;
    uint32_t tc_blk_attr_mask = 0;
    bool mel_clip_attr_set = false;
    uint32_t tc_attr_mask = 0;
    bool tc_heads = true;
    int* d_peer_err = nullptr;
    bool grp_heads = true;
    struct oww_heads_grp* heads_grp = nullptr;
    int tc_heads_terms = 3;
    struct oww_detector* det = nullptr;
    struct oww_audio* audio = nullptr;
    struct oww_ingest_state* ingest = nullptr;
    struct oww_clip_resampler* clip_rs = nullptr;
};

int oww_fail(oww_ctx* ctx, int code, const char* fmt, ...);
void oww_verifier_fit_free(oww_ctx* ctx);
inline uint64_t oww_fnv1a(const void* p, size_t bytes, uint64_t h = 14695981039346656037ull) {
    const unsigned char* c = static_cast<const unsigned char*>(p);
    for (size_t i = 0; i < bytes; ++i) h = (h ^ c[i]) * 1099511628211ull;
    return h;
}
#define OWW_CUDA(ctx, call)                                                                    \
    do {                                                                                       \
        cudaError_t e__ = (call);                                                              \
        if (e__ != cudaSuccess)                                                                \
            return oww_fail((ctx), OWW_ECUDA, "%s failed: %s (%s:%d)", #call,                  \
                            cudaGetErrorString(e__), __FILE__, __LINE__);                      \
    } while (0)
#ifdef __CUDACC__
template <typename... KArgs, typename... Args>
inline cudaError_t oww_launch_pdl(bool pdl, void (*kernel)(KArgs...), dim3 grid, dim3 block, size_t smem, cudaStream_t s, Args&&... args) {
    cudaLaunchConfig_t cfg = {};
    cfg.gridDim = grid; cfg.blockDim = block; cfg.dynamicSmemBytes = smem; cfg.stream = s;
    cudaLaunchAttribute at[1];
    at[0].id = cudaLaunchAttributeProgrammaticStreamSerialization;
    at[0].val.programmaticStreamSerializationAllowed = pdl ? 1 : 0;
    cfg.attrs = at; cfg.numAttrs = 1;
    return cudaLaunchKernelEx(&cfg, kernel, std::forward<Args>(args)...);
}
__device__ __forceinline__ void oww_pdl_sync() {
    asm volatile("griddepcontrol.launch_dependents;" ::: "memory");
    asm volatile("griddepcontrol.wait;" ::: "memory");
}
#endif

#define OWW_LAUNCH_CHECK(ctx)                                                                  \
    do {                                                                                       \
        (ctx)->launches++;                                                                     \
        cudaError_t e__ = cudaGetLastError();                                                  \
        if (e__ != cudaSuccess)                                                                \
            return oww_fail((ctx), OWW_ECUDA, "kernel launch failed: %s (%s:%d)",              \
                            cudaGetErrorString(e__), __FILE__, __LINE__);                      \
    } while (0)

#ifdef __CUDACC__
#define OWW_HD __host__ __device__ __forceinline__
#else
#define OWW_HD inline
#endif
OWW_HD int64_t oww_clip_calls(int64_t L, int c) { return L > c ? (L - 1) / c : 0; }
OWW_HD int64_t oww_call_first_step(int64_t j, int c) { return j * c / OWW_SAMPLES_PER_CHUNK; }
OWW_HD int64_t oww_call_of_step(int64_t s, int c) { return ((int64_t)OWW_SAMPLES_PER_CHUNK * (s + 1) + c - 1) / c - 1; }

struct MelLaunch {
    const int16_t* body; int64_t body_stride; int n_body;
    int16_t* tail;
    int* seen;
    float* out; int64_t out_stride; int out_rows_mask;
    int* out_count;
    int n_clips; int affine; int n_chunks;
    const int* ids = nullptr;
    const int* live = nullptr;
    int live_min = 0;
    bool pdl = false;
};
int oww_mel_launch(oww_ctx* ctx, const MelLaunch& p, cudaStream_t s);
int oww_mel_clips_launch(oww_ctx* ctx, const int16_t* d_pcm, const int64_t* d_off, const int* d_len, int n_clips, int pad,
                         int chunk, int k0, int k1, float* d_out, int64_t out_stride, cudaStream_t s);

struct WindowSrc {
    const float* base; int64_t stride;
    const int* count; int rows_mask;
    int n_streams; int n_chunks;
    const int* ids = nullptr;
};
int oww_feat_append(oww_ctx* ctx, const float* d_emb, int n_chunks, cudaStream_t s, const int* d_ids = nullptr, int n_ids = 0);
int oww_cnn_window(oww_ctx* ctx, const WindowSrc& src, int n_windows, float* d_emb, cudaStream_t s, bool capture_tails = false);
int oww_cnn_fp32_pyramid(oww_ctx* ctx, const WindowSrc& src, int n, int T0, float* d_emb, int out_rows, int stop_layer,
                         float* d_dbg, cudaStream_t s);

int oww_tc_pack_weights(oww_ctx* ctx, const float* h_blob);
size_t oww_tc_act_units(const oww_ctx* ctx, int n_windows);
size_t oww_tc_act_units_T(const oww_ctx* ctx, int n, int T0);
int oww_late_alloc(oww_ctx* ctx);
int oww_late_chain(oww_ctx* ctx, float* d_emb, cudaStream_t s);
int oww_late_capture(oww_ctx* ctx, int next_layer, const void* planes, int64_t plane_pitch, int T, int W, cudaStream_t s);
int oww_cnn_tc_pyramid(oww_ctx* ctx, const WindowSrc& src, int n, int T0, float* d_emb, int out_rows, int stop_layer,
                       float* d_dbg, cudaStream_t s);
struct TailCapture { int win0, n_win, stream0; const int* ids = nullptr; bool late = false; };
int oww_cnn_tc_pyramid_cap(oww_ctx* ctx, const WindowSrc& src, int n, float* d_emb, const TailCapture* cap, cudaStream_t s);

int oww_inc_build_plan(oww_ctx* ctx, int G, int n_streams, int n_layers, IncPlan* out);
int oww_inc_n_layers(const oww_ctx* ctx);
int oww_inc_setup(oww_ctx* ctx, const float* h_blob);
int oww_inc_alloc_streams(oww_ctx* ctx);
int oww_cnn_inc_step(oww_ctx* ctx, int back, float* d_emb, cudaStream_t s, const int* d_chunks = nullptr, int min_chunks = 0);
bool oww_fused_frontend_supported(const oww_ctx* ctx);
bool oww_fused_heads_supported(const oww_ctx* ctx);
int oww_fused_step(oww_ctx* ctx, const int16_t* d_pcm, int64_t pcm_stride, float* d_scores, int out_stride, bool with_heads,
                   cudaStream_t s, const int* d_chunks = nullptr, int min_chunks = 0);
int oww_heads_sync_devs(oww_ctx* ctx);
int oww_inc_capture(oww_ctx* ctx, int layer, const void* planes, int64_t plane_pitch, int T, int W, int win0, int n_win,
                    int stream0, const int* d_ids, cudaStream_t s);

struct FeatSrc {
    const float* base; int64_t stride;
    const int* count; int rows_mask;
    int back;
    int steps = 0, row0 = 0;
    const int* idx = nullptr;
};
#ifdef __CUDACC__
struct FeatRows { const float* base; int r0, mask; };
__device__ __forceinline__ FeatRows feat_rows(const FeatSrc& src, int n_in, int s) {
    if (src.count) return FeatRows{src.base + (int64_t)s * src.stride, src.count[s] - src.back - n_in, src.rows_mask};
    if (src.steps > 0) {
        const int q = src.idx ? src.idx[s] : s;
        const int clip = q / src.steps, st = q - clip * src.steps;
        return FeatRows{src.base + (int64_t)clip * src.stride, src.row0 + st + 1 - n_in, -1};
    }
    return FeatRows{src.base + (int64_t)s * src.stride, 0, -1};
}
__device__ __forceinline__ const float* feat_row(const FeatRows& w, int c) {
    const int r = w.r0 + c;
    return r < 0 ? nullptr : w.base + (int64_t)(w.mask >= 0 ? (r & w.mask) : r) * 96;
}
#endif
int oww_heads_launch(oww_ctx* ctx, int head_id, const FeatSrc& src, int n, float* d_out, int out_stride,
                     int out_col0, int combine_max, cudaStream_t s, uint32_t head_mask = 0xFFFFFFFFu);

int oww_check_head_desc(oww_ctx* ctx, const oww_head_desc* desc);
int oww_stage_head(oww_ctx* ctx, const oww_head_desc* desc, const float* h_blob, size_t n_floats, Head& h,
                   std::vector<float>& staged);

int oww_heads_tc_pack(oww_ctx* ctx, Head& h, const float* w1);
struct BankRows { const int4* items; const int* perm; int n_items; };
int oww_head_banks_launch(oww_ctx* ctx, const FeatSrc& src, int n, float* d_out, int out_stride, int combine_max,
                          cudaStream_t s, const int* d_step = nullptr, const BankRows* rows = nullptr);
const int* oww_head_bank_stream_slots(const oww_ctx* ctx, int bank);
int oww_head_banks_alloc_streams(oww_ctx* ctx);
void oww_head_banks_free(oww_ctx* ctx);
bool oww_heads_tc_supported(const oww_ctx* ctx, int head_id);
int oww_heads_tc_launch(oww_ctx* ctx, int head_id, const FeatSrc& src, int n, float* d_out, int out_stride,
                        int out_col0, int combine_max, cudaStream_t s, uint32_t head_mask = 0xFFFFFFFFu);
void oww_heads_grp_free(oww_ctx* ctx);
void oww_heads_grp_drop_mirror(oww_ctx* ctx);
void oww_feat16_invalidate(oww_ctx* ctx);
int oww_feat16_advance(oww_ctx* ctx, int n_chunks, cudaStream_t s);
int oww_feat16_resync(oww_ctx* ctx, const int* d_ids, int n, cudaStream_t s);
uint32_t oww_heads_grp_covered(oww_ctx* ctx);
uint32_t oww_heads_grp_bulk(oww_ctx* ctx, const FeatSrc& src, int n, float* d_out, int out_stride, cudaStream_t s, int* rc_out);
int oww_heads_grp_launch(oww_ctx* ctx, int back, int n, float* d_out, int out_stride, int combine_max, cudaStream_t s);
int oww_heads_all(oww_ctx* ctx, const FeatSrc& src, int n, float* d_out, int out_stride, int combine_max, cudaStream_t s,
                  const BankRows* bank_rows = nullptr);

void oww_detect_free(oww_ctx* ctx);
void oww_detect_free_streams(oww_ctx* ctx);
int oww_detect_alloc_streams(oww_ctx* ctx);
int oww_detect_reset(oww_ctx* ctx, const int* d_ids, int n, cudaStream_t s);

void oww_audio_free(oww_ctx* ctx);
void oww_audio_free_streams(oww_ctx* ctx);
int oww_audio_alloc_streams(oww_ctx* ctx);
int oww_audio_reset(oww_ctx* ctx, const int* d_ids, int n, cudaStream_t s);
int oww_audio_append(oww_ctx* ctx, const int16_t* d_pcm, int64_t pcm_stride, int n_chunks, const int* d_counts,
                     cudaStream_t s);

void oww_ingest_free(oww_ctx* ctx);
void oww_ingest_free_streams(oww_ctx* ctx);
int oww_ingest_alloc_streams(oww_ctx* ctx);
void oww_ingest_reset(oww_ctx* ctx, const int32_t* h_ids, int n);

int oww_verifiers_apply(oww_ctx* ctx, const FeatSrc& src, int n, float* d_scores, int out_stride, bool clips,
                        cudaStream_t s, const int* d_chunks = nullptr, const int* d_clip_streams = nullptr);
int oww_verifiers_alloc_streams(oww_ctx* ctx);
bool oww_verifiers_clip_active(const oww_ctx* ctx, bool clip_streams = false);
void oww_verifiers_free_streams(oww_ctx* ctx);
```

Measured before the change: 6.238 million.

## Replace shared-memory mel FFT with register/shuffle FFT and pack clips per CTA

The 512-point real FFT used for mel frames now runs in registers with warp shuffles (radix-8 in-thread, then xor-shuffle stages) instead of radix-4 passes through shared memory. Per-lane window and twiddle values are preloaded and mel weights are transposed for coalesced loads. The standalone mel kernel is restructured into a persistent grid that packs several clips per CTA, with an occupancy-derived split of frames across warps. This targets shared-memory traffic, syncwarps and launch/occupancy overhead in the mel frontend, at the cost of more registers per thread and a changed weight and twiddle layout.

```diff
diff --git a/openwakeword_b200/csrc/cnn_tc_inc.cu b/openwakeword_b200/csrc/cnn_tc_inc.cu
--- a/openwakeword_b200/csrc/cnn_tc_inc.cu
+++ b/openwakeword_b200/csrc/cnn_tc_inc.cu
@@ -10,7 +10,6 @@
 constexpr int kIncEpiWarps = 16;
 constexpr int kIncThreads = kIncEpiWarps * 32;
 constexpr int kIncMaxG = 7;
-constexpr int kMelNF = 2;
 
 __device__ __forceinline__ __half2 u32_as_half2(uint32_t v) {
     return __halves2half2(__ushort_as_half((unsigned short)(v & 0xFFFFu)), __ushort_as_half((unsigned short)(v >> 16)));
@@ -114,7 +113,7 @@
         uint4* tout = a.tails_out + (int64_t)grp * P.tail_units;
         int* s_cnt = reinterpret_cast<int*>(smem + 512);
         int* s_live = s_cnt + 16;
-        float* s_mel = reinterpret_cast<float*>(smem + P.scratch_off + 6144);
+        float* s_mel = reinterpret_cast<float*>(smem + P.scratch_off);
         if (a.dbg_clock && blockIdx.x == 0 && grp == 0 && et == 0) a.dbg_clock[101] = clock64();
         named_bar_sync(2, kIncEpiWarps * 32);
         if (et < G) {
@@ -123,13 +122,9 @@
         }
         named_bar_sync(2, kIncEpiWarps * 32);
         if (fused) {
-            uint8_t* sc = smem + P.scratch_off;
-            float2* s_tw = reinterpret_cast<float2*>(sc);
-            float* s_win = reinterpret_cast<float*>(sc + 4096);
-            uint8_t* s_work = smem + 2048 + warp * (kMelNF * kMelFrameScratch);
+            float* s_pw = reinterpret_cast<float*>(smem + 2048 + warp * kMelPwBytes);
             float* s_floor = s_mel + G * 256;
             int seen_v = 1;
-            for (int i = et; i < 512; i += kIncEpiWarps * 32) { s_tw[i] = a.mel_twiddle[i]; s_win[i] = a.mel_window[i]; }
             if (et < G) {
                 const int b = grp * G + et;
                 s_cnt[et] = s_live[et] ? a.mel_count_rw[b] : 0;
@@ -139,21 +134,15 @@
             }
             named_bar_sync(2, kIncEpiWarps * 32);
             const int my_start = a.mel_start[lane], my_len = a.mel_len[lane];
-            const float* my_w = a.mel_w + lane * OWW_MEL_MAXSUPPORT;
-            for (int fi = warp * kMelNF; fi < G * 8; fi += kIncEpiWarps * kMelNF) {
-                const int16_t* tl[kMelNF]; const int16_t* bd[kMelNF]; int fr[kMelNF]; float db[kMelNF];
-#pragma unroll
-                for (int i = 0; i < kMelNF; ++i) {
-                    const int fj = fi + i < G * 8 ? fi + i : fi;
-                    int b = grp * G + (fj >> 3);
-                    if (b >= a.B) b = grp * G;
-                    tl[i] = a.tail + (int64_t)b * OWW_TAIL; bd[i] = a.pcm + (int64_t)b * a.pcm_stride; fr[i] = fj & 7;
-                }
+            const float* my_w = a.mel_w + lane;
+            const MelLane L = mel_lane_load(a.mel_window, a.mel_twiddle, lane);
+#pragma unroll 1
+            for (int fi = warp; fi < G * 8; fi += kIncEpiWarps) {
+                int b = grp * G + (fi >> 3);
+                if (b >= a.B) b = grp * G;
                 long long* st = (a.dbg_clock && blockIdx.x == 0 && grp == 0 && warp == 0 && fi == 0) ? a.dbg_clock + 92 : nullptr;
-                mel_frames_db<kMelNF>(tl, OWW_TAIL, bd, fr, s_work, s_tw, s_win, a.mel_kmax, my_start, my_len, my_w, lane, db, st);
-#pragma unroll
-                for (int i = 0; i < kMelNF; ++i)
-                    if (fi + i < G * 8) s_mel[(fi + i) * 32 + lane] = db[i];
+                s_mel[fi * 32 + lane] = mel_frame(L, a.tail + (int64_t)b * OWW_TAIL, OWW_TAIL, a.pcm + (int64_t)b * a.pcm_stride,
+                                                  fi & 7, s_pw, a.mel_kmax, my_start, my_len, my_w, lane, st);
             }
             named_bar_sync(2, kIncEpiWarps * 32);
             if (a.dbg_clock && blockIdx.x == 0 && grp == 0 && et == 0) a.dbg_clock[97] = clock64();
@@ -823,9 +812,9 @@
     }
     if (NL == OWW_N_CONV) {
         int off = kActBase + r8(size_nx[0]) * 16;
-        const int work_end = kActBase + kIncEpiWarps * kMelNF * kMelFrameScratch;
+        const int work_end = kActBase + kIncEpiWarps * kMelPwBytes;
         if (work_end > off) off = (work_end + 127) & ~127;
-        const int need_b = 6144 + G * 256 * 4 + 64;
+        const int need_b = G * 256 * 4 + 64;
         P.scratch_off = (off + need_b <= P.L[1].w_smem && off + need_b <= P.L[2].w_smem) ? off : 0;
     }
     P.w_total_bytes = (int)w_off;
diff --git a/openwakeword_b200/csrc/mel.cu b/openwakeword_b200/csrc/mel.cu
--- a/openwakeword_b200/csrc/mel.cu
+++ b/openwakeword_b200/csrc/mel.cu
@@ -9,6 +9,7 @@
 
 constexpr int kWarps = 8;
 constexpr int kThreads = kWarps * 32;
+constexpr int kKeep = 8;
 
 struct MelDev {
     const float* window;
@@ -19,93 +20,89 @@
     int kmax;
 };
 
-__global__ void __launch_bounds__(kThreads, 5) mel_kernel(MelLaunch p, MelDev c) {
-    __shared__ __align__(16) uint8_t s_work[kWarps][kMelFrameScratch];
-    __shared__ float2 s_tw[512];
-    __shared__ float s_win[512];
-    __shared__ float s_red[kWarps];
+__global__ void __launch_bounds__(kThreads, 2) mel_kernel(MelLaunch p, MelDev c, int spi) {
+    __shared__ __align__(16) float s_pw[kWarps][kMelPwFloats];
+    __shared__ float s_red[2][kWarps];
+    __shared__ float s_keep[kWarps][kKeep][32];
 
     pdl_trigger();
-    const int clip = p.ids ? p.ids[blockIdx.x] : blockIdx.x;
-    const int tid = threadIdx.x, lane = tid & 31, warp = tid >> 5;
-    if (p.live && p.live[clip] < p.live_min) {
-        pdl_wait();
-        return;
-    }
-
-    for (int i = tid; i < 512; i += kThreads) { s_tw[i] = c.twiddle[i]; s_win[i] = c.window[i]; }
-
+    const int lane = threadIdx.x & 31, warp = threadIdx.x >> 5;
+    const MelLane L = mel_lane_load(c.window, c.twiddle, lane);
+    const int my_start = c.mel_start[lane];
+    const int my_len = c.mel_len[lane];
+    const float* my_w = c.mel_w + lane;
+
+    const int ipc = kWarps / spi;
+    const int slot = warp / spi, sub = warp - slot * spi;
     const bool streaming = p.tail != nullptr;
     const int prefix = streaming ? OWW_TAIL : 0;
-    const int seen0 = streaming ? p.seen[clip] : 0;
-    const bool fresh = streaming && seen0 == 0;
-    const int total = prefix + p.n_body;
-    const int T = (total - OWW_FFT_N) / OWW_HOP + 1;
-    const int f0 = fresh ? 3 : 0;
-    const int nrows = T - f0;
-    const bool one_pass = nrows <= kWarps;
-    const int16_t* body = p.body + (int64_t)clip * p.body_stride;
-    const int16_t* tail = streaming ? p.tail + (int64_t)clip * OWW_TAIL : nullptr;
-    const int row0 = p.out_count ? p.out_count[clip] : 0;
-    float* out = p.out + (int64_t)clip * p.out_stride;
-    __syncthreads();
-
-    const int my_start = c.mel_start[lane];
-    const int my_len = c.mel_len[lane];
-    const float* my_w = c.mel_w + lane * OWW_MEL_MAXSUPPORT;
-    float vmax = -INFINITY, kept = 0.f;
-
-    for (int f = f0 + warp; f < T; f += kWarps) {
-        float db;
-        mel_frames_db<1>(&tail, prefix, &body, &f, s_work[warp], s_tw, s_win, c.kmax, my_start, my_len, my_w, lane, &db);
-        vmax = fmaxf(vmax, db);
-        if (one_pass) { kept = db; continue; }
+    const int T = (prefix + p.n_body - OWW_FFT_N) / OWW_HOP + 1;
+    int par = 0;
+    for (int base = blockIdx.x * ipc; base < p.n_clips; base += gridDim.x * ipc, par ^= 1) {
+        const int j = base + slot;
+        bool active = j < p.n_clips;
+        const int clip = active ? (p.ids ? p.ids[j] : j) : 0;
+        if (active && p.live && p.live[clip] < p.live_min) active = false;
+        const int seen0 = active && streaming ? p.seen[clip] : 0;
+        const bool fresh = streaming && seen0 == 0;
+        const int f0 = fresh ? 3 : 0;
+        const int nrows = T - f0;
+        const bool one_pass = nrows <= kKeep * spi;
+        const int16_t* body = p.body + (int64_t)clip * p.body_stride;
+        const int16_t* tail = streaming ? p.tail + (int64_t)clip * OWW_TAIL : nullptr;
+        const int row0 = active && p.out_count ? p.out_count[clip] : 0;
+        float* out = p.out + (int64_t)clip * p.out_stride;
+
+        float vmax = -INFINITY;
+        if (active) {
+#pragma unroll 1
+            for (int i = 0, f = f0 + sub; f < T; ++i, f += spi) {
+                const float db = mel_frame(L, tail, prefix, body, f, s_pw[warp], c.kmax, my_start, my_len, my_w, lane);
+                vmax = fmaxf(vmax, db);
+                if (one_pass) { s_keep[warp][i][lane] = db; continue; }
+                pdl_wait();
+                const int r = f - f0;
+                const int slot_r = p.out_rows_mask >= 0 ? ((row0 + r) & p.out_rows_mask) : r;
+                out[(int64_t)slot_r * OWW_MEL_BINS + lane] = db;
+            }
+        }
+#pragma unroll
+        for (int o = 16; o > 0; o >>= 1) vmax = fmaxf(vmax, __shfl_xor_sync(0xffffffffu, vmax, o));
+        if (spi > 1) {
+            if (lane == 0) s_red[par][warp] = vmax;
+            __syncthreads();
+            for (int w = 0; w < spi; ++w) vmax = fmaxf(vmax, s_red[par][slot * spi + w]);
+        }
+        const float floor_db = vmax - 80.0f;
         pdl_wait();
-        const int r = f - f0;
-        const int slot = p.out_rows_mask >= 0 ? ((row0 + r) & p.out_rows_mask) : r;
-        out[(int64_t)slot * OWW_MEL_BINS + lane] = db;
-    }
-#pragma unroll
-    for (int o = 16; o > 0; o >>= 1) vmax = fmaxf(vmax, __shfl_xor_sync(0xffffffffu, vmax, o));
-    if (lane == 0) s_red[warp] = vmax;
-    __syncthreads();
-    float m = s_red[0];
-#pragma unroll
-    for (int w = 1; w < kWarps; ++w) m = fmaxf(m, s_red[w]);
-    const float floor_db = m - 80.0f;
-    int16_t tv[(OWW_TAIL + kThreads - 1) / kThreads];
-#pragma unroll
-    for (int u = 0; u < (OWW_TAIL + kThreads - 1) / kThreads; ++u) {
-        const int i = tid + u * kThreads;
-        tv[u] = streaming && i < OWW_TAIL ? __ldg(body + (p.n_body - OWW_TAIL + i)) : (int16_t)0;
-    }
-    pdl_wait();
-    if (one_pass) {
-        if (warp < nrows) {
-            float v = fmaxf(kept, floor_db);
-            if (p.affine) v = v / 10.0f + 2.0f;
-            const int slot = p.out_rows_mask >= 0 ? ((row0 + warp) & p.out_rows_mask) : warp;
-            out[(int64_t)slot * OWW_MEL_BINS + lane] = v;
-        }
-    } else {
-        for (int i = tid; i < nrows * OWW_MEL_BINS; i += kThreads) {
-            const int r = i >> 5, col = i & 31;
-            const int slot = p.out_rows_mask >= 0 ? ((row0 + r) & p.out_rows_mask) : r;
-            float* q = out + (int64_t)slot * OWW_MEL_BINS + col;
-            float v = fmaxf(__ldcg(q), floor_db);
-            if (p.affine) v = v / 10.0f + 2.0f;
-            *q = v;
-        }
-    }
-    if (streaming) {
-        int16_t* tw = p.tail + (int64_t)clip * OWW_TAIL;
-#pragma unroll
-        for (int u = 0; u < (OWW_TAIL + kThreads - 1) / kThreads; ++u)
-            if (tid + u * kThreads < OWW_TAIL) tw[tid + u * kThreads] = tv[u];
-        if (tid == 0) {
-            p.out_count[clip] = oww_wrap_count(row0 + nrows);
-            const int sn = seen0 + p.n_chunks;
-            p.seen[clip] = sn > (1 << 30) ? (1 << 30) : sn;
+        if (!active) continue;
+        if (one_pass) {
+            for (int u = 0; u < kKeep; ++u) {
+                const int r = sub + u * spi;
+                if (r < nrows) {
+                    float v = fmaxf(s_keep[warp][u][lane], floor_db);
+                    if (p.affine) v = v / 10.0f + 2.0f;
+                    const int slot_r = p.out_rows_mask >= 0 ? ((row0 + r) & p.out_rows_mask) : r;
+                    out[(int64_t)slot_r * OWW_MEL_BINS + lane] = v;
+                }
+            }
+        } else {
+            for (int r = sub; r < nrows; r += spi) {
+                const int slot_r = p.out_rows_mask >= 0 ? ((row0 + r) & p.out_rows_mask) : r;
+                float* q = out + (int64_t)slot_r * OWW_MEL_BINS + lane;
+                float v = fmaxf(*q, floor_db);
+                if (p.affine) v = v / 10.0f + 2.0f;
+                *q = v;
+            }
+        }
+        if (streaming) {
+            int16_t* tw = p.tail + (int64_t)clip * OWW_TAIL;
+            for (int i = sub * 32 + lane; i < OWW_TAIL; i += spi * 32) tw[i] = __ldg(body + (p.n_body - OWW_TAIL + i));
+            if (sub == 0 && lane == 0) {
+                p.out_count[clip] = oww_wrap_count(row0 + nrows);
+                const int sn = seen0 + p.n_chunks;
+                p.seen[clip] = sn > (1 << 30) ? (1 << 30) : sn;
+            }
         }
     }
 }
@@ -119,11 +116,8 @@
 __global__ void __launch_bounds__(kThreads) mel_clip_kernel(const int16_t* pcm, const int64_t* clip_off, const int* clip_len, int pad,
                                                             int chunk, int k0, int k1, float* out, int64_t out_stride, MelDev c) {
     extern __shared__ __align__(16) uint8_t dyn[];
-    float2 (*s_buf)[2][256] = reinterpret_cast<float2 (*)[2][256]>(dyn);
-    float2* s_tw = reinterpret_cast<float2*>(dyn + kWarps * 2 * 256 * sizeof(float2));
-    float* s_win = reinterpret_cast<float*>(s_tw + 512);
-    float (*s_pow)[264] = reinterpret_cast<float (*)[264]>(s_win + 512);
-    int16_t (*s_frame)[512] = reinterpret_cast<int16_t (*)[512]>(s_pow + kWarps);
+    float (*s_pw)[kMelPwFloats] = reinterpret_cast<float (*)[kMelPwFloats]>(dyn);
+    int16_t (*s_frame)[512] = reinterpret_cast<int16_t (*)[512]>(s_pw + kWarps);
     int* s_gmax = reinterpret_cast<int*>(s_frame + kWarps);
     const int clip = blockIdx.x;
     const int tid = threadIdx.x, lane = tid & 31, warp = tid >> 5;
@@ -131,16 +125,16 @@
     const int g0 = clip_first_group(k0, chunk);
     const int f0 = g0 == 0 ? 0 : 8 * g0 - 3;
     const int n_frames = 8 * k1 - 3;
-    for (int i = tid; i < 512; i += kThreads) { s_tw[i] = c.twiddle[i]; s_win[i] = c.window[i]; }
     for (int i = tid; i < k1 - g0; i += kThreads) s_gmax[i] = INT_MIN;
     const int16_t* body = pcm + clip_off[clip];
     const int n_samples = clip_len[clip];
     float* o = out + (int64_t)clip * out_stride;
     for (int i = tid; i < (71 - v0) * 32; i += kThreads) o[i] = 1.0f;
     __syncthreads();
+    const MelLane L = mel_lane_load(c.window, c.twiddle, lane);
     const int my_start = c.mel_start[lane];
     const int my_len = c.mel_len[lane];
-    const float* my_w = c.mel_w + lane * OWW_MEL_MAXSUPPORT;
+    const float* my_w = c.mel_w + lane;
     auto enc = [](float v) { int i = __float_as_int(v); return i >= 0 ? i : i ^ 0x7FFFFFFF; };
     for (int f = f0 + warp; f < n_frames; f += kWarps) {
         for (int j = lane; j < 512; j += 32) {
@@ -148,8 +142,7 @@
             s_frame[warp][j] = (p >= 0 && p < n_samples) ? body[p] : (int16_t)0;
         }
         __syncwarp();
-        const float db = mel_frame_db<false>(nullptr, 0, s_frame[warp], 0, s_buf[warp][0], s_buf[warp][1], s_pow[warp], s_tw, s_win, c.kmax,
-                                      my_start, my_len, my_w, lane);
+        const float db = mel_frame<false>(L, nullptr, 0, s_frame[warp], 0, s_pw[warp], c.kmax, my_start, my_len, my_w, lane);
         if (71 + f >= v0) o[(int64_t)(71 + f - v0) * 32 + lane] = db;
         float m = db;
 #pragma unroll
@@ -187,7 +180,19 @@
     if (prefix + p.n_body < OWW_FFT_N) return oww_fail(ctx, OWW_EINVAL, "clip shorter than 512 samples");
     if (p.n_clips <= 0) return OWW_OK;
     MelDev c{ctx->d_window, ctx->d_twiddle, ctx->d_mel_start, ctx->d_mel_len, ctx->d_mel_w, ctx->mel_kmax};
-    OWW_CUDA(ctx, oww_launch_pdl(p.pdl, mel_kernel, dim3(p.n_clips), dim3(kThreads), 0, s, p, c));
+    if (ctx->mel_ctas_per_sm == 0) {
+        int n = 0;
+        OWW_CUDA(ctx, cudaOccupancyMaxActiveBlocksPerMultiprocessor(&n, mel_kernel, kThreads, 0));
+        ctx->mel_ctas_per_sm = n > 0 ? n : 1;
+    }
+    const int slots = ctx->sm_count * ctx->mel_ctas_per_sm;
+    const int T = (prefix + p.n_body - OWW_FFT_N) / OWW_HOP + 1;
+    int spi = 1;
+    while (spi < kWarps && spi < T && (int64_t)p.n_clips * spi < (int64_t)slots * kWarps) spi *= 2;
+    const int ipc = kWarps / spi;
+    const int64_t need = ((int64_t)p.n_clips + ipc - 1) / ipc;
+    const int grid = (int)need;
+    OWW_CUDA(ctx, oww_launch_pdl(p.pdl, mel_kernel, dim3(grid), dim3(kThreads), 0, s, p, c, spi));
     OWW_LAUNCH_CHECK(ctx);
     return OWW_OK;
 }
@@ -199,8 +204,7 @@
     if (k0 < 0 || k1 - k0 > 8192 || chunk < 1 || oww_call_first_step(oww_call_of_step(k1, chunk), chunk) != k1)
         return oww_fail(ctx, OWW_EINVAL, "step range [%d,%d) is not a bulk frontend segment", k0, k1);
     MelDev c{ctx->d_window, ctx->d_twiddle, ctx->d_mel_start, ctx->d_mel_len, ctx->d_mel_w, ctx->mel_kmax};
-    const size_t smem = (size_t)kWarps * 2 * 256 * sizeof(float2) + 512 * sizeof(float2) + 512 * sizeof(float) +
-                        (size_t)kWarps * 264 * sizeof(float) + (size_t)kWarps * 512 * sizeof(int16_t) +
+    const size_t smem = (size_t)kWarps * kMelPwBytes + (size_t)kWarps * 512 * sizeof(int16_t) +
                         (size_t)(k1 - clip_first_group(k0, chunk)) * sizeof(int);
     if (!ctx->mel_clip_attr_set) {
         OWW_CUDA(ctx, cudaFuncSetAttribute(mel_clip_kernel, cudaFuncAttributeMaxDynamicSharedMemorySize, 100 * 1024));
@@ -221,11 +225,18 @@
     } else {
         for (int n = 0; n < 400; ++n) win[56 + n] = (float)(0.5 - 0.5 * std::cos(2.0 * kPi * n / 400.0));
     }
-    std::vector<float2> tw(512);
+    std::vector<float2> tw(512 + 512);
     for (int k = 0; k < 512; ++k) {
         const double a = -2.0 * kPi * k / 512.0;
         tw[k] = make_float2((float)std::cos(a), (float)std::sin(a));
     }
+    for (int k1 = 0; k1 < 8; ++k1)
+        for (int l = 0; l < 32; ++l) {
+            int n0 = 0;
+            for (int b = 0; b < 5; ++b) n0 |= ((l >> b) & 1) << (4 - b);
+            tw[512 + 32 * k1 + l] = tw[k1 + 8 * l];
+            tw[768 + 32 * k1 + l] = tw[(2 * n0 * k1) & 511];
+        }
     std::vector<float> fb(OWW_N_BINS * OWW_MEL_BINS);
     if (h_mel_fb) {
         std::memcpy(fb.data(), h_mel_fb, fb.size() * sizeof(float));
@@ -258,7 +269,7 @@
             return oww_fail(ctx, OWW_EUNSUPPORTED, "mel filter %d spans %d FFT bins (max %d)", i, hi - lo + 1,
                             OWW_MEL_MAXSUPPORT);
         st[i] = lo; ln[i] = hi - lo + 1;
-        for (int k = lo; k <= hi; ++k) mw[i * OWW_MEL_MAXSUPPORT + (k - lo)] = fb[k * OWW_MEL_BINS + i];
+        for (int k = lo; k <= hi; ++k) mw[(k - lo) * OWW_MEL_BINS + i] = fb[k * OWW_MEL_BINS + i];
         if (hi + 1 > kmax) kmax = hi + 1;
     }
     ctx->mel_kmax = kmax;
@@ -268,7 +279,7 @@
         return cudaMemcpy(*d, h, bytes, cudaMemcpyHostToDevice);
     };
     OWW_CUDA(ctx, up((void**)&ctx->d_window, win.data(), 512 * sizeof(float)));
-    OWW_CUDA(ctx, up((void**)&ctx->d_twiddle, tw.data(), 512 * sizeof(float2)));
+    OWW_CUDA(ctx, up((void**)&ctx->d_twiddle, tw.data(), tw.size() * sizeof(float2)));
     OWW_CUDA(ctx, up((void**)&ctx->d_mel_start, st.data(), OWW_MEL_BINS * sizeof(int)));
     OWW_CUDA(ctx, up((void**)&ctx->d_mel_len, ln.data(), OWW_MEL_BINS * sizeof(int)));
     OWW_CUDA(ctx, up((void**)&ctx->d_mel_w, mw.data(), mw.size() * sizeof(float)));
diff --git a/openwakeword_b200/csrc/mel_device.cuh b/openwakeword_b200/csrc/mel_device.cuh
--- a/openwakeword_b200/csrc/mel_device.cuh
+++ b/openwakeword_b200/csrc/mel_device.cuh
@@ -8,205 +8,131 @@
 __device__ __forceinline__ float2 cmul(float2 a, float2 b) {
     return make_float2(__fmaf_rn(a.x, b.x, -__fmul_rn(a.y, b.y)), __fmaf_rn(a.x, b.y, __fmul_rn(a.y, b.x)));
 }
+__device__ __forceinline__ float2 cadd(float2 a, float2 b) { return make_float2(__fadd_rn(a.x, b.x), __fadd_rn(a.y, b.y)); }
+__device__ __forceinline__ float2 csub(float2 a, float2 b) { return make_float2(__fsub_rn(a.x, b.x), __fsub_rn(a.y, b.y)); }
+__device__ __forceinline__ float2 mul_mi(float2 a) { return make_float2(a.y, -a.x); }
+__device__ __forceinline__ float2 shfl_xor2(float2 v, int m) {
+    return make_float2(__shfl_xor_sync(0xffffffffu, v.x, m), __shfl_xor_sync(0xffffffffu, v.y, m));
+}
+
+__device__ __forceinline__ void dft4(float2& c0, float2& c1, float2& c2, float2& c3) {
+    const float2 e0 = cadd(c0, c2), e1 = csub(c0, c2), e2 = cadd(c1, c3), e3 = mul_mi(csub(c1, c3));
+    c0 = cadd(e0, e2); c1 = cadd(e1, e3); c2 = csub(e0, e2); c3 = csub(e1, e3);
+}
+
+struct MelLane {
+    float2 win[8];
+    const float2* tw8;
+    float2 tws[4];
+    const float2* twu;
+};
+
+__device__ __forceinline__ MelLane mel_lane_load(const float* window, const float2* twiddle, int lane) {
+    MelLane L;
+    const int n0 = (int)(__brev((unsigned)lane) >> 27);
+#pragma unroll
+    for (int j = 0; j < 8; ++j) L.win[j] = __ldg(reinterpret_cast<const float2*>(window) + n0 + 32 * j);
+    L.tw8 = twiddle + 768 + lane;
+#pragma unroll
+    for (int s = 0; s < 4; ++s) {
+        const int h = 2 << s;
+        L.tws[s] = (lane & h) ? __ldg(twiddle + (lane & (h - 1)) * (256 / h)) : make_float2(1.f, 0.f);
+    }
+    L.twu = twiddle + 512 + lane;
+    return L;
+}
+
+constexpr int kMelPwFloats = 264;
+constexpr int kMelPwBytes = kMelPwFloats * 4;
 
 template <bool kBodyGlobal = true>
-__device__ __forceinline__ float mel_frame_db(const int16_t* tail, int prefix, const int16_t* body, int f, float2* a, float2* b,
-                                              float* pw_buf, const float2* s_tw, const float* s_win, int kmax, int my_start,
-                                              int my_len, const float* my_w, int lane) {
+__device__ __forceinline__ float mel_frame(const MelLane& L, const int16_t* tail, int prefix, const int16_t* body, int f,
+                                           float* pw, int kmax, int my_start, int my_len, const float* my_w, int lane,
+                                           long long* stamps = nullptr) {
+    if (stamps && lane == 0) stamps[0] = clock64();
+    const int n0 = (int)(__brev((unsigned)lane) >> 27);
+    const bool al = (((size_t)body | (size_t)tail) & 3) == 0 && (prefix & 1) == 0;
+    uint32_t raw[8];
 #pragma unroll
-        for (int j = 0; j < 8; ++j) {
-            const int n = lane + 32 * j;
-            const int s0 = f * OWW_HOP + 2 * n;
-            float x0, x1;
-            if (s0 + 1 < prefix) { x0 = (float)tail[s0]; x1 = (float)tail[s0 + 1]; }
+    for (int j = 0; j < 8; ++j) {
+        const int s0 = f * OWW_HOP + 2 * (n0 + 32 * j);
+        if (al) {
+            const uint32_t* bp = reinterpret_cast<const uint32_t*>(body + (s0 - prefix));
+            raw[j] = s0 + 1 < prefix ? *reinterpret_cast<const uint32_t*>(tail + s0) : (kBodyGlobal ? __ldg(bp) : *bp);
+        } else {
+            unsigned short u0, u1;
+            if (s0 + 1 < prefix) { u0 = (unsigned short)tail[s0]; u1 = (unsigned short)tail[s0 + 1]; }
             else if (s0 >= prefix) {
-                if (kBodyGlobal) { x0 = (float)__ldg(body + (s0 - prefix)); x1 = (float)__ldg(body + (s0 + 1 - prefix)); }
-                else { x0 = (float)body[s0 - prefix]; x1 = (float)body[s0 + 1 - prefix]; }
+                const int16_t* q = body + (s0 - prefix);
+                u0 = (unsigned short)(kBodyGlobal ? __ldg(q) : q[0]); u1 = (unsigned short)(kBodyGlobal ? __ldg(q + 1) : q[1]);
             }
-            else { x0 = (float)tail[s0]; x1 = kBodyGlobal ? (float)__ldg(body) : (float)body[0]; }
-            a[n] = make_float2(__fmul_rn(x0, s_win[2 * n]), __fmul_rn(x1, s_win[2 * n + 1]));
+            else { u0 = (unsigned short)tail[s0]; u1 = (unsigned short)(kBodyGlobal ? __ldg(body) : body[0]); }
+            raw[j] = (uint32_t)u0 | ((uint32_t)u1 << 16);
         }
-        __syncwarp();
+    }
+    float2 z[8];
 #pragma unroll
-        for (int Ns = 1; Ns < 256; Ns *= 4) {
-            const int tstep = 128 / Ns;
+    for (int j = 0; j < 8; ++j) {
+        const float x0 = (float)(short)(raw[j] & 0xFFFFu), x1 = (float)(short)(raw[j] >> 16);
+        z[j] = make_float2(__fmul_rn(x0, L.win[j].x), __fmul_rn(x1, L.win[j].y));
+    }
+    if (stamps && lane == 0) stamps[1] = clock64();
+    {
+        const float c = 0.70710678118654752f;
+        float2 a[4], b[4];
 #pragma unroll
-            for (int jj = 0; jj < 2; ++jj) {
-                const int j = lane + 32 * jj;
-                const int k = j & (Ns - 1);
-                float2 v0 = a[j];
-                float2 v1 = cmul(a[j + 64], s_tw[k * tstep]);
-                float2 v2 = cmul(a[j + 128], s_tw[2 * k * tstep]);
-                float2 v3 = cmul(a[j + 192], s_tw[3 * k * tstep]);
-                float2 a0 = make_float2(v0.x + v2.x, v0.y + v2.y);
-                float2 a1 = make_float2(v0.x - v2.x, v0.y - v2.y);
-                float2 a2 = make_float2(v1.x + v3.x, v1.y + v3.y);
-                float2 d = make_float2(v1.x - v3.x, v1.y - v3.y);
-                float2 a3 = make_float2(d.y, -d.x);
-                const int dst = (j / Ns) * Ns * 4 + k;
-                b[dst] = make_float2(a0.x + a2.x, a0.y + a2.y);
-                b[dst + Ns] = make_float2(a1.x + a3.x, a1.y + a3.y);
-                b[dst + 2 * Ns] = make_float2(a0.x - a2.x, a0.y - a2.y);
-                b[dst + 3 * Ns] = make_float2(a1.x - a3.x, a1.y - a3.y);
-            }
-            __syncwarp();
-            float2* t = a; a = b; b = t;
+        for (int j = 0; j < 4; ++j) { a[j] = cadd(z[j], z[j + 4]); b[j] = csub(z[j], z[j + 4]); }
+        b[1] = make_float2(__fmul_rn(c, __fadd_rn(b[1].x, b[1].y)), __fmul_rn(c, __fsub_rn(b[1].y, b[1].x)));
+        b[2] = mul_mi(b[2]);
+        b[3] = make_float2(__fmul_rn(c, __fsub_rn(b[3].y, b[3].x)), -__fmul_rn(c, __fadd_rn(b[3].x, b[3].y)));
+        dft4(a[0], a[1], a[2], a[3]);
+        dft4(b[0], b[1], b[2], b[3]);
+#pragma unroll
+        for (int m = 0; m < 4; ++m) { z[2 * m] = a[m]; z[2 * m + 1] = b[m]; }
+    }
+#pragma unroll
+    for (int k1 = 1; k1 < 8; ++k1) z[k1] = cmul(z[k1], __ldg(L.tw8 + 32 * k1));
+#pragma unroll
+    for (int s = 0; s < 5; ++s) {
+        const int h = 1 << s;
+        const float sg = (lane & h) ? -1.f : 1.f;
+#pragma unroll
+        for (int k1 = 0; k1 < 8; ++k1) {
+            const float2 q = s == 0 ? z[k1] : cmul(z[k1], L.tws[s - 1]);
+            const float2 p = shfl_xor2(q, h);
+            z[k1] = make_float2(__fmaf_rn(sg, q.x, p.x), __fmaf_rn(sg, q.y, p.y));
         }
-        for (int k = lane; k < kmax; k += 32) {
-            float pw;
-            if (k == 256) {
-                const float x = a[0].x - a[0].y;
-                pw = __fmul_rn(x, x);
-            } else {
-                const float2 zk = a[k & 255];
-                const float2 zc = a[(256 - k) & 255];
-                const float2 xe = make_float2(0.5f * (zk.x + zc.x), 0.5f * (zk.y - zc.y));
-                const float2 dd = make_float2(zk.x - zc.x, zk.y + zc.y);
-                const float2 xo = make_float2(0.5f * dd.y, -0.5f * dd.x);
-                const float2 t2 = cmul(s_tw[k], xo);
-                const float re = __fadd_rn(xe.x, t2.x), im = __fadd_rn(xe.y, t2.y);
-                pw = __fmaf_rn(re, re, __fmul_rn(im, im));
-            }
-            pw_buf[k] = pw;
-        }
-        __syncwarp();
-        float acc = 0.f;
-        for (int i = 0; i < my_len; ++i) acc = fmaf(pw_buf[my_start + i], my_w[i], acc);
-        const float db = 10.0f * logf(fmaxf(acc, 1e-10f)) / logf(10.0f);
+    }
+    if (stamps && lane == 0) stamps[2] = clock64();
+    float2 zc[8];
+    zc[0] = make_float2(__shfl_sync(0xffffffffu, z[0].x, (32 - lane) & 31), __shfl_sync(0xffffffffu, z[0].y, (32 - lane) & 31));
+#pragma unroll
+    for (int k1 = 1; k1 < 8; ++k1) zc[8 - k1] = shfl_xor2(z[k1], 31);
+    float p8[8];
+#pragma unroll
+    for (int k1 = 0; k1 < 8; ++k1) {
+        const float2 zk = z[k1];
+        const float2 xe = make_float2(__fmul_rn(0.5f, __fadd_rn(zk.x, zc[k1].x)), __fmul_rn(0.5f, __fsub_rn(zk.y, zc[k1].y)));
+        const float2 dd = make_float2(__fsub_rn(zk.x, zc[k1].x), __fadd_rn(zk.y, zc[k1].y));
+        const float2 xo = make_float2(__fmul_rn(0.5f, dd.y), __fmul_rn(-0.5f, dd.x));
+        const float2 t2 = cmul(__ldg(L.twu + 32 * k1), xo);
+        const float re = __fadd_rn(xe.x, t2.x), im = __fadd_rn(xe.y, t2.y);
+        p8[k1] = __fmaf_rn(re, re, __fmul_rn(im, im));
+    }
+    reinterpret_cast<float4*>(pw)[2 * lane] = make_float4(p8[0], p8[1], p8[2], p8[3]);
+    reinterpret_cast<float4*>(pw)[2 * lane + 1] = make_float4(p8[4], p8[5], p8[6], p8[7]);
+    if (lane == 0 && kmax > 256) {
+        const float x = __fsub_rn(z[0].x, z[0].y);
+        pw[256] = __fmul_rn(x, x);
+    }
+    __syncwarp();
+    if (stamps && lane == 0) stamps[3] = clock64();
+    float acc = 0.f;
+    for (int q = 0; q < my_len; ++q) acc = __fmaf_rn(pw[my_start + q], __ldg(my_w + 32 * q), acc);
+    const float db = 10.0f * logf(fmaxf(acc, 1e-10f)) / logf(10.0f);
+    __syncwarp();
+    if (stamps && lane == 0) stamps[4] = clock64();
     return db;
 }
 
-#ifndef OWW_FFT_SWZ
-#define OWW_FFT_SWZ 1
-#endif
-__device__ __forceinline__ int fswz(int e) {
-#if OWW_FFT_SWZ
-    return e ^ (((e >> 4) & 3) * 5);
-#else
-    return e;
-#endif
 }
-
-constexpr int kMelFrameScratch = 2048 + 2048;
-template <int NF>
-__device__ __forceinline__ void mel_frames_db(const int16_t* const* tail, int prefix, const int16_t* const* body, const int* f,
-                                              uint8_t* bufs, const float2* s_tw, const float* s_win, int kmax, int my_start,
-                                              int my_len, const float* my_w, int lane, float* db, long long* stamps = nullptr) {
-    float2* a[NF]; float2* b[NF]; float* pw[NF];
-    if (stamps && lane == 0) stamps[0] = clock64();
-#pragma unroll
-    for (int i = 0; i < NF; ++i) {
-        a[i] = reinterpret_cast<float2*>(bufs + i * kMelFrameScratch);
-        b[i] = a[i] + 256;
-        pw[i] = reinterpret_cast<float*>(b[i]);
-    }
-    bool al[NF];
-#pragma unroll
-    for (int i = 0; i < NF; ++i) al[i] = (((size_t)body[i] | (size_t)tail[i]) & 3) == 0 && (prefix & 1) == 0;
-    uint32_t raw[8][NF];
-#pragma unroll
-    for (int j = 0; j < 8; ++j) {
-        const int n = lane + 32 * j;
-#pragma unroll
-        for (int i = 0; i < NF; ++i) {
-            const int s0 = f[i] * OWW_HOP + 2 * n;
-            if (al[i]) {
-                raw[j][i] = s0 + 1 < prefix ? *reinterpret_cast<const uint32_t*>(tail[i] + s0)
-                                            : __ldg(reinterpret_cast<const uint32_t*>(body[i] + (s0 - prefix)));
-            } else {
-                unsigned short u0, u1;
-                if (s0 + 1 < prefix) { u0 = (unsigned short)tail[i][s0]; u1 = (unsigned short)tail[i][s0 + 1]; }
-                else if (s0 >= prefix) { u0 = (unsigned short)__ldg(body[i] + (s0 - prefix)); u1 = (unsigned short)__ldg(body[i] + (s0 + 1 - prefix)); }
-                else { u0 = (unsigned short)tail[i][s0]; u1 = (unsigned short)__ldg(body[i]); }
-                raw[j][i] = (uint32_t)u0 | ((uint32_t)u1 << 16);
-            }
-        }
-    }
-#pragma unroll
-    for (int j = 0; j < 8; ++j) {
-        const int n = lane + 32 * j;
-        const float2 wn = *reinterpret_cast<const float2*>(s_win + 2 * n);
-#pragma unroll
-        for (int i = 0; i < NF; ++i) {
-            const float x0 = (float)(short)(raw[j][i] & 0xFFFFu), x1 = (float)(short)(raw[j][i] >> 16);
-            a[i][fswz(n)] = make_float2(__fmul_rn(x0, wn.x), __fmul_rn(x1, wn.y));
-        }
-    }
-    __syncwarp();
-    if (stamps && lane == 0) stamps[1] = clock64();
-#pragma unroll
-    for (int Ns = 1; Ns < 256; Ns *= 4) {
-        const int tstep = 128 / Ns;
-        float2 t1 = make_float2(1.f, 0.f), t2 = t1, t3 = t1;
-        if (Ns > 1 && Ns <= 32) { const int k = lane & (Ns - 1); t1 = s_tw[k * tstep]; t2 = s_tw[2 * k * tstep]; t3 = s_tw[3 * k * tstep]; }
-#pragma unroll
-        for (int jj = 0; jj < 2; ++jj) {
-            const int j = lane + 32 * jj;
-            const int k = j & (Ns - 1);
-            if (Ns > 32) { t1 = s_tw[k * tstep]; t2 = s_tw[2 * k * tstep]; t3 = s_tw[3 * k * tstep]; }
-            const int dst = (j / Ns) * Ns * 4 + k;
-            const int sj = fswz(j);
-            const int d0 = fswz(dst), d1 = fswz(dst + Ns), d2 = fswz(dst + 2 * Ns), d3 = fswz(dst + 3 * Ns);
-#pragma unroll
-            for (int i = 0; i < NF; ++i) {
-                const float2 v0 = a[i][sj];
-                float2 v1 = a[i][sj + 64], v2 = a[i][sj + 128], v3 = a[i][sj + 192];
-                if (Ns > 1) { v1 = cmul(v1, t1); v2 = cmul(v2, t2); v3 = cmul(v3, t3); }
-                float2 a0 = make_float2(v0.x + v2.x, v0.y + v2.y);
-                float2 a1 = make_float2(v0.x - v2.x, v0.y - v2.y);
-                float2 a2 = make_float2(v1.x + v3.x, v1.y + v3.y);
-                float2 d = make_float2(v1.x - v3.x, v1.y - v3.y);
-                float2 a3 = make_float2(d.y, -d.x);
-                b[i][d0] = make_float2(a0.x + a2.x, a0.y + a2.y);
-                b[i][d1] = make_float2(a1.x + a3.x, a1.y + a3.y);
-                b[i][d2] = make_float2(a0.x - a2.x, a0.y - a2.y);
-                b[i][d3] = make_float2(a1.x - a3.x, a1.y - a3.y);
-            }
-        }
-        __syncwarp();
-#pragma unroll
-        for (int i = 0; i < NF; ++i) { float2* t = a[i]; a[i] = b[i]; b[i] = t; }
-    }
-    if (stamps && lane == 0) stamps[2] = clock64();
-    for (int k = lane; k < kmax; k += 32) {
-#pragma unroll
-        for (int i = 0; i < NF; ++i) {
-            float p;
-            if (k == 256) {
-                const float x = a[i][fswz(0)].x - a[i][fswz(0)].y;
-                p = __fmul_rn(x, x);
-            } else {
-                const float2 zk = a[i][fswz(k & 255)];
-                const float2 zc = a[i][fswz((256 - k) & 255)];
-                const float2 xe = make_float2(0.5f * (zk.x + zc.x), 0.5f * (zk.y - zc.y));
-                const float2 dd = make_float2(zk.x - zc.x, zk.y + zc.y);
-                const float2 xo = make_float2(0.5f * dd.y, -0.5f * dd.x);
-                const float2 t2 = cmul(s_tw[k], xo);
-                const float re = __fadd_rn(xe.x, t2.x), im = __fadd_rn(xe.y, t2.y);
-                p = __fmaf_rn(re, re, __fmul_rn(im, im));
-            }
-            pw[i][k] = p;
-        }
-    }
-    __syncwarp();
-    if (stamps && lane == 0) stamps[3] = clock64();
-    float acc[NF];
-#pragma unroll
-    for (int i = 0; i < NF; ++i) acc[i] = 0.f;
-    for (int q = 0; q < my_len; q += 4) {
-        const float4 w4 = __ldg(reinterpret_cast<const float4*>(my_w + q));
-        const float w[4] = {w4.x, w4.y, w4.z, w4.w};
-#pragma unroll
-        for (int e = 0; e < 4; ++e)
-            if (q + e < my_len) {
-#pragma unroll
-                for (int i = 0; i < NF; ++i) acc[i] = fmaf(pw[i][my_start + q + e], w[e], acc[i]);
-            }
-    }
-#pragma unroll
-    for (int i = 0; i < NF; ++i) db[i] = 10.0f * logf(fmaxf(acc[i], 1e-10f)) / logf(10.0f);
-    __syncwarp();
-    if (stamps && lane == 0) stamps[4] = clock64();
-}
-
-}
diff --git a/openwakeword_b200/csrc/oww_internal.h b/openwakeword_b200/csrc/oww_internal.h
--- a/openwakeword_b200/csrc/oww_internal.h
+++ b/openwakeword_b200/csrc/oww_internal.h
@@ -262,6 +262,7 @@
     bool heads_tc_attr_set = false;
     uint32_t tc_blk_attr_mask = 0;
     bool mel_clip_attr_set = false;
+    int mel_ctas_per_sm = 0;
     uint32_t tc_attr_mask = 0;
     bool tc_heads = true;
     int* d_peer_err = nullptr;
```

New measurement: 6.291 million, median of 6. No clear change (+0.8%).
